# PKU-VCL-Geometry/GeoSplatting

Measured on AMD Instinct MI355X. Metric: fwd+bwd views/sec at 2M Gaussians, 800x800, higher is better.
Workload: dtype f32

## Files before the change

geosplatting_amd/_lib.py:

```python
from __future__ import annotations

import ctypes as C
import os
from typing import Optional

import torch

_HERE = os.path.dirname(os.path.abspath(__file__))
LIB_PATH = os.path.join(_HERE, "libgeosplat_hip.so")

GS_MAX_LEVELS = 16


class GsEnv(C.Structure):
    _fields_ = [("lut", C.c_void_p), ("lut_res", C.c_int), ("base", C.c_void_p), ("base_res", C.c_int),
                ("num_levels", C.c_int), ("levels", C.c_void_p * GS_MAX_LEVELS), ("res", C.c_int * GS_MAX_LEVELS),
                ("min_roughness", C.c_float), ("max_roughness", C.c_float)]


class GsTailView(C.Structure):
    _fields_ = [("viewmat", C.c_void_p), ("K", C.c_void_p), ("cam_pos", C.c_void_p), ("vis_records", C.c_void_p), ("v_packed", C.c_void_p),
                ("packed_index", C.c_void_p), ("W", C.c_int), ("H", C.c_int)]


class GsTileLevel(C.Structure):
    _fields_ = [("R", C.c_int), ("n_mirrors", C.c_int), ("margin", C.c_int), ("bw", C.c_int), ("nb", C.c_int), ("tile_begin", C.c_int),
                ("tile_end", C.c_int), ("reserved", C.c_int), ("src", C.c_void_p), ("scale", C.c_void_p), ("out_scale", C.c_void_p),
                ("bounds", C.c_void_p), ("tiles", C.c_void_p), ("segments", C.c_void_p), ("row_begin", C.c_void_p), ("row_counts", C.c_void_p),
                ("desc", C.c_void_p), ("weights", C.c_void_p), ("dst", C.c_void_p), ("lds_bytes", C.c_size_t)]


class GsEnvGrad(C.Structure):
    _fields_ = [("base", C.c_void_p), ("levels", C.c_void_p * GS_MAX_LEVELS)]


SYMBOLS = [
    "gs_last_error", "gs_version", "gs_project_ws_bytes", "gs_project_fwd", "gs_project_fwd_vis", "gs_project_fwd_vis_ex", "gs_isect_emit", "gs_sort_ws_bytes",
    "gs_isect_sort", "gs_isect_bin_ws_bytes", "gs_isect_bin", "gs_isect_offsets", "gs_raster_ws_bytes", "gs_raster_fwd", "gs_raster_prepare", "gs_raster_prepare_vis", "gs_raster_composite", "gs_raster_grad_stride", "gs_raster_bwd", "gs_raster_bwd_acc", "gs_selftest_rcp", "gs_selftest_exp", "gs_selftest_cube_edges", "gs_isect_bin_cap", "gs_isect_offsets_cap", "gs_isect_bin_tiles_cap", "gs_isect_offsets_tiles_cap", "gs_raster_prepare_vis_cap", "gs_raster_composite_cap", "gs_raster_bwd_cap", "gs_raster_bwd_acc_cap", "gs_raster_composite_tone", "gs_raster_bwd_tone_acc", "gs_raster_log_ws_bytes", "gs_raster_composite_tone_log", "gs_raster_bwd_tone_log_acc", "gs_project_bwd_cap", "gs_project_bwd", "gs_project_bwd_ex", "gs_shade_fwd",
    "gs_shade_bwd_ws_bytes", "gs_shade_bwd", "gs_tonemap_fwd", "gs_tonemap_bwd", "gs_tonemap_fwd3", "gs_tonemap_bwd3", "gs_cubemap_mip_fwd", "gs_cubemap_mip_chain_fwd", "gs_cube_sample_linear",
    "gs_cubemap_mip_bwd", "gs_diffuse_cubemap_fwd", "gs_diffuse_cubemap_bwd", "gs_specular_bounds", "gs_specular_bounds_ws_bytes", "gs_specular_bounds_fast", "gs_cube_dir_table",
    "gs_specular_cubemap_fwd", "gs_specular_cubemap_bwd", "gs_specular_tiles_count", "gs_specular_tiles_fill",
    "gs_specular_tiles_check", "gs_specular_tiles_apply", "gs_specular_tiles_apply_multi", "gs_mgadapter_fwd", "gs_mgadapter_bwd", "gs_vertex_normals_fwd",
    "gs_vertex_normals_bwd", "gs_photo_loss_ws_bytes", "gs_photo_loss", "gs_hashgrid_fwd", "gs_hashgrid_bwd_ws_bytes", "gs_hashgrid_bwd", "gs_hashgrid_bwd_fixed_ws_bytes", "gs_hashgrid_bwd_fixed", "gs_mlp_wgrad_ws_bytes", "gs_mlp_wgrad",
    "gs_flexicubes_ws_bytes", "gs_flexicubes_count", "gs_flexicubes_fwd", "gs_flexicubes_bwd", "gs_flexicubes_entropy_fwd",
    "gs_flexicubes_entropy_bwd", "gs_front_ws_bytes", "gs_front_fwd", "gs_isect_bin_front_ws_bytes", "gs_isect_bin_front", "gs_tail_bwd", "gs_tail_bwd_multi", "gs_tail_bwd_multi_parts", "gs_tail_priv_ws_bytes", "gs_tail_priv_reduce", "gs_activation_chain",
]

_lib: Optional[C.CDLL] = None


class GeoSplatHipError(RuntimeError):
    pass


def lib() -> C.CDLL:
    global _lib
    if _lib is None:
        if not os.path.exists(LIB_PATH):
            raise GeoSplatHipError(
                f"{LIB_PATH} not found: build it with `python -m geosplatting_amd.build` "
                "(hipcc --offload-arch=gfx950).  geosplatting_amd has no CPU / PyTorch fallback.")
        l = C.CDLL(LIB_PATH)
        l.gs_last_error.restype = C.c_char_p
        l.gs_project_ws_bytes.restype = C.c_size_t
        l.gs_project_ws_bytes.argtypes = [C.c_int]
        l.gs_sort_ws_bytes.restype = C.c_size_t
        l.gs_sort_ws_bytes.argtypes = [C.c_int64, C.c_int, C.c_int]
        l.gs_isect_bin_ws_bytes.restype = C.c_size_t
        l.gs_isect_bin_ws_bytes.argtypes = [C.c_int, C.c_int64, C.c_int, C.c_int]
        l.gs_shade_bwd_ws_bytes.restype = C.c_size_t
        l.gs_shade_bwd_ws_bytes.argtypes = [C.c_void_p, C.c_int]
        l.gs_hashgrid_bwd_ws_bytes.restype = C.c_size_t
        l.gs_hashgrid_bwd_ws_bytes.argtypes = [C.c_int, C.c_int, C.c_int]
        l.gs_hashgrid_bwd_fixed_ws_bytes.restype = C.c_size_t
        l.gs_hashgrid_bwd_fixed_ws_bytes.argtypes = [C.c_int, C.c_int, C.c_int, C.c_int]
        l.gs_mlp_wgrad_ws_bytes.restype = C.c_size_t
        l.gs_mlp_wgrad_ws_bytes.argtypes = [C.c_int64]
        l.gs_flexicubes_ws_bytes.restype = C.c_size_t
        l.gs_flexicubes_ws_bytes.argtypes = [C.c_int, C.c_int, C.c_int]
        l.gs_photo_loss_ws_bytes.restype = C.c_size_t
        l.gs_photo_loss_ws_bytes.argtypes = [C.c_int, C.c_int]
        l.gs_specular_bounds_ws_bytes.restype = C.c_size_t
        l.gs_specular_bounds_ws_bytes.argtypes = [C.c_int]
        l.gs_front_ws_bytes.restype = C.c_size_t
        l.gs_front_ws_bytes.argtypes = [C.c_int]
        l.gs_isect_bin_front_ws_bytes.restype = C.c_size_t
        l.gs_isect_bin_front_ws_bytes.argtypes = [C.c_int, C.c_int64, C.c_int, C.c_int]
        l.gs_tail_priv_ws_bytes.restype = C.c_size_t
        l.gs_tail_priv_ws_bytes.argtypes = [C.c_void_p, C.c_int]
        l.gs_raster_log_ws_bytes.restype = C.c_size_t
        l.gs_raster_log_ws_bytes.argtypes = [C.c_int64, C.c_int, C.c_int, C.c_int]
        l.gs_raster_ws_bytes.restype = C.c_size_t
        l.gs_raster_ws_bytes.argtypes = [C.c_int64, C.c_int, C.c_int, C.c_int, C.c_int]
        _lib = l
    return _lib


def check(rc: int, what: str) -> None:
    if rc != 0:
        raise GeoSplatHipError(f"{what} failed ({rc}): {lib().gs_last_error().decode()}")


def ptr(t: Optional[torch.Tensor]) -> Optional[C.c_void_p]:
    if t is None:
        return None
    assert t.is_cuda and t.is_contiguous(), "device-resident contiguous tensors only"
    return C.c_void_p(t.data_ptr())


def stream() -> C.c_void_p:
    return C.c_void_p(torch.cuda.current_stream().cuda_stream)


def f32(x: float) -> C.c_float:
    return C.c_float(float(x))


def i64(x: int) -> C.c_int64:
    return C.c_int64(int(x))


def require_cuda(*tensors: torch.Tensor) -> None:
    for t in tensors:
        if t is not None and not t.is_cuda:
            raise GeoSplatHipError("geosplatting_amd ops run on the GPU only (tensor on %s); there is no CPU path" % t.device)


_shared_streams = {}


def shared_stream(device: torch.device, role: str) -> "torch.cuda.Stream":
    key = (device.index if device.index is not None else torch.cuda.current_device(), role)
    st = _shared_streams.get(key)
    if st is None:
        st = _shared_streams[key] = torch.cuda.Stream(device=device)
    return st
```

geosplatting_amd/csrc/gs_common.h:

```cpp
#pragma once
#include <hip/hip_runtime.h>
#include <stdint.h>
#include <stdio.h>

#include "../../include/geosplat_hip.h"

#define GS_WAVE 64

void gs_set_error(const char* fmt, ...);

#define GS_CHECK_ARG(cond, msg)                                  \
    do {                                                         \
        if (!(cond)) { gs_set_error("%s: %s", __func__, msg); return GS_EINVAL; } \
    } while (0)

#define GS_CHECK_HIP(expr)                                                              \
    do {                                                                                \
        hipError_t _e = (expr);                                                         \
        if (_e != hipSuccess) {                                                         \
            gs_set_error("%s: %s failed: %s", __func__, #expr, hipGetErrorString(_e));  \
            return GS_ELAUNCH;                                                          \
        }                                                                               \
    } while (0)

#define GS_CHECK_LAUNCH()  GS_CHECK_HIP(hipGetLastError())

static inline int gs_cdiv(int64_t a, int64_t b) { return (int)((a + b - 1) / b); }

struct GsCount {
    long long n;
    const long long* dev;
};
__device__ __forceinline__ long long gs_count(const GsCount& c)
{
    if (c.dev == nullptr) return c.n;
    const long long v = *c.dev;
    return v < 0 ? 0 : (v < c.n ? v : c.n);
}

static __global__ void __launch_bounds__(256) gs_zero_kernel(uint32_t* __restrict__ p, size_t n_words)
{
    for (size_t i = (size_t)blockIdx.x * blockDim.x + threadIdx.x; i < n_words; i += (size_t)gridDim.x * blockDim.x) p[i] = 0u;
}
static __global__ void __launch_bounds__(256) gs_zero16_kernel(uint4* __restrict__ p, size_t n_quads)
{
    for (size_t i = (size_t)blockIdx.x * blockDim.x + threadIdx.x; i < n_quads; i += (size_t)gridDim.x * blockDim.x) p[i] = make_uint4(0u, 0u, 0u, 0u);
}
static inline hipError_t gs_zero_async(void* p, size_t bytes, hipStream_t s)
{
    if (bytes == 0) return hipSuccess;
    if ((bytes & 3) != 0 || (((uintptr_t)p) & 3) != 0) return hipMemsetAsync(p, 0, bytes, s);
    const bool wide = (bytes & 15) == 0 && (((uintptr_t)p) & 15) == 0;
    const size_t n = wide ? bytes / 16 : bytes / 4;
    const size_t want = (n + 255) / 256;
    const int blocks = (int)(want < 4096 ? want : 4096);
    if (wide) hipLaunchKernelGGL(gs_zero16_kernel, dim3(blocks), dim3(256), 0, s, (uint4*)p, n);
    else hipLaunchKernelGGL(gs_zero_kernel, dim3(blocks), dim3(256), 0, s, (uint32_t*)p, n);
    return hipGetLastError();
}

__device__ __forceinline__ float gs_readlane(float v, int lane)
{
    return __builtin_bit_cast(float, __builtin_amdgcn_readlane(__builtin_bit_cast(int, v), lane));
}
__device__ __forceinline__ int gs_readlane(int v, int lane) { return __builtin_amdgcn_readlane(v, lane); }

template <int CTRL, int ROW_MASK, int BANK_MASK>
__device__ __forceinline__ float gs_dpp_add(float v)
{
    int o = __builtin_amdgcn_update_dpp(0, __builtin_bit_cast(int, v), CTRL, ROW_MASK, BANK_MASK, false);
    return v + __builtin_bit_cast(float, o);
}

__device__ __forceinline__ float gs_wave_sum(float v)
{
    v = gs_dpp_add<0xB1, 0xf, 0xf>(v);
    v = gs_dpp_add<0x4E, 0xf, 0xf>(v);
    v = gs_dpp_add<0x141, 0xf, 0xf>(v);
    v = gs_dpp_add<0x140, 0xf, 0xf>(v);
    v = gs_dpp_add<0x142, 0xa, 0xf>(v);
    v = gs_dpp_add<0x143, 0xc, 0xf>(v);
    return gs_readlane(v, 63);
}

template <int CTRL, int ROW_MASK>
__device__ __forceinline__ unsigned gs_dpp_add_u32(unsigned v)
{
    return v + (unsigned)__builtin_amdgcn_update_dpp(0, (int)v, CTRL, ROW_MASK, 0xf, false);
}
__device__ __forceinline__ unsigned gs_wave_incl_scan(unsigned v)
{
    v = gs_dpp_add_u32<0x111, 0xf>(v);
    v = gs_dpp_add_u32<0x112, 0xf>(v);
    v = gs_dpp_add_u32<0x114, 0xf>(v);
    v = gs_dpp_add_u32<0x118, 0xf>(v);
    v = gs_dpp_add_u32<0x142, 0xa>(v);
    v = gs_dpp_add_u32<0x143, 0xc>(v);
    return v;
}
__device__ __forceinline__ int gs_wave_incl_scan(int v) { return (int)gs_wave_incl_scan((unsigned)v); }
__device__ __forceinline__ unsigned gs_wave_sum_u32(unsigned v)
{
    v = gs_dpp_add_u32<0xB1, 0xf>(v);
    v = gs_dpp_add_u32<0x4E, 0xf>(v);
    v = gs_dpp_add_u32<0x141, 0xf>(v);
    v = gs_dpp_add_u32<0x140, 0xf>(v);
    v = gs_dpp_add_u32<0x142, 0xa>(v);
    v = gs_dpp_add_u32<0x143, 0xc>(v);
    return (unsigned)__builtin_amdgcn_readlane((int)v, 63);
}
__device__ __forceinline__ unsigned long long gs_wave_sum_u64(unsigned long long v)
{
    const unsigned a = gs_wave_sum_u32((unsigned)(v & 0x1fffffull)), b = gs_wave_sum_u32((unsigned)((v >> 21) & 0x1fffffull)),
                   c = gs_wave_sum_u32((unsigned)(v >> 42));
    return (unsigned long long)a + ((unsigned long long)b << 21) + ((unsigned long long)c << 42);
}

template <int CTRL>
__device__ __forceinline__ float gs_dpp_take(float give)
{
    return __builtin_bit_cast(float, __builtin_amdgcn_update_dpp(0, __builtin_bit_cast(int, give), CTRL, 0xf, 0xf, true));
}

template <int N, int CTRL>
__device__ __forceinline__ void gs_bfly_stage(const float* in, float* out, bool own_hi)
{
#pragma unroll
    for (int z = 0; z < (N + 1) / 2; ++z) {
        const float lo = in[2 * z];
        const float hi = (2 * z + 1 < N) ? in[2 * z + 1] : 0.0f;
        const float keep = own_hi ? hi : lo;
        const float give = own_hi ? lo : hi;
        out[z] = keep + gs_dpp_take<CTRL>(give);
    }
}

template <int NV>
struct GsBfly {
    static constexpr int N1 = (NV + 1) / 2, N2 = (N1 + 1) / 2, N3 = (N2 + 1) / 2, N4 = (N3 + 1) / 2;
    __device__ static __forceinline__ int owned_index(int lane, int q)
    {
        return 16 * q + 8 * (lane & 1) + 4 * ((lane >> 1) & 1) + 2 * ((lane >> 2) & 1) + ((lane >> 3) & 1);
    }
    __device__ static __forceinline__ void reduce_rows(const float (&v)[NV], float (&out)[N4], int lane)
    {
        float a[N1], b[N2], c[N3];
        gs_bfly_stage<NV, 0x140>(v, a, (lane & 8) != 0);
        gs_bfly_stage<N1, 0x141>(a, b, (lane & 4) != 0);
        gs_bfly_stage<N2, 0x4E>(b, c, (lane & 2) != 0);
        gs_bfly_stage<N3, 0xB1>(c, out, (lane & 1) != 0);
    }
    __device__ static __forceinline__ void reduce(const float (&v)[NV], float (&out)[N4], int lane)
    {
        float a[N1], b[N2], c[N3];
        gs_bfly_stage<NV, 0x140>(v, a, (lane & 8) != 0);
        gs_bfly_stage<N1, 0x141>(a, b, (lane & 4) != 0);
        gs_bfly_stage<N2, 0x4E>(b, c, (lane & 2) != 0);
        gs_bfly_stage<N3, 0xB1>(c, out, (lane & 1) != 0);
#pragma unroll
        for (int q = 0; q < N4; ++q) {
            out[q] += __shfl_xor(out[q], 16, 64);
            out[q] += __shfl_xor(out[q], 32, 64);
        }
    }
};

__device__ __forceinline__ float gs_exp_neg(float sigma)
{
#pragma clang fp contract(off)
    const float y = sigma * -1.44269504f;
    const float yc = fminf(fmaxf(y, -126.0f), 126.0f);
    const float n = __builtin_rintf(yc);
    const float f = yc - n;
    float p = 0x1.41a6fep-13f;
    p = __builtin_fmaf(p, f, 0x1.5f44f0p-10f);
    p = __builtin_fmaf(p, f, 0x1.3b2dfep-7f);
    p = __builtin_fmaf(p, f, 0x1.c6aed6p-5f);
    p = __builtin_fmaf(p, f, 0x1.ebfbdap-3f);
    p = __builtin_fmaf(p, f, 0x1.62e430p-1f);
    p = __builtin_fmaf(p, f, 1.0f);
    const float r = __builtin_ldexpf(p, (int)n);
    return (y >= -125.0f) ? r : 0.0f;
}

__device__ __forceinline__ bool alpha_extent(float ca, float cb, float cc, float o, float& hx, float& hy)
{
    const float tau = __logf(255.0f * o);
    const float det = ca * cc - cb * cb;
    if (!(tau > -0.002f)) return false;
    if (!(det > 0.0f)) { hx = hy = 1e30f; return true; }
    const float k = 2.0f * (tau + 0.002f) / det;
    hx = sqrtf(k * cc) * 1.0005f + 0.02f;
    hy = sqrtf(k * ca) * 1.0005f + 0.02f;
    return true;
}

__device__ __forceinline__ void gs_write_vis_record(float4* __restrict__ rec, float mx, float my, float ca, float cb, float cc, float op,
                                                    float c0, float c1, float c2)
{
    float hx = -1.0f, hy = -1.0f;
    if (!alpha_extent(ca, cb, cc, op, hx, hy)) { hx = -1.0f; hy = -1.0f; }
    rec[0] = make_float4(mx, my, 0.5f * ca, cb);
    rec[1] = make_float4(0.5f * cc, op, hx, hy);
    rec[2] = make_float4(c0, c1, c2, 0.0f);
    rec[3] = make_float4(0.f, 0.f, 0.f, 0.f);
}

__device__ __forceinline__ int gs_lane_id() { return (int)(threadIdx.x & 63); }

__device__ __forceinline__ void gs_atomic_add(float* p, float v) { unsafeAtomicAdd(p, v); }

__device__ __forceinline__ void gs_atomic_add_xcd(float* p, float v)
{
    __hip_atomic_fetch_add(p, v, __ATOMIC_RELAXED, __HIP_MEMORY_SCOPE_WORKGROUP);
}

__device__ __forceinline__ int gs_xcc_id()
{
    return (int)(__builtin_amdgcn_s_getreg((3 << 11) | (0 << 6) | 20) & 0xf);
}
```

geosplatting_amd/csrc/gs_raster.hip:

```cpp
#include "gs_common.h"
#include "gs_tone.h"
#include <stdlib.h>

#pragma clang fp contract(off)

#define GS_TILE 16
#define GS_ALPHA_MIN (1.0f / 255.0f)

#ifdef GS_RASTER_STATS
__device__ unsigned long long g_raster_stats[8];
extern "C" int gs_raster_stats_read(unsigned long long* host8, int reset)
{
    if (hipMemcpyFromSymbol(host8, HIP_SYMBOL(g_raster_stats), sizeof(unsigned long long) * 8) != hipSuccess) return -1;
    if (reset) { unsigned long long z[8] = {0}; if (hipMemcpyToSymbol(HIP_SYMBOL(g_raster_stats), z, sizeof(z)) != hipSuccess) return -1; }
    return 0;
}
__device__ unsigned long long g_raster_stats2[8];
extern "C" int gs_raster_stats2_read(unsigned long long* host8, int reset)
{
    if (hipMemcpyFromSymbol(host8, HIP_SYMBOL(g_raster_stats2), sizeof(unsigned long long) * 8) != hipSuccess) return -1;
    if (reset) { unsigned long long z[8] = {0}; if (hipMemcpyToSymbol(HIP_SYMBOL(g_raster_stats2), z, sizeof(z)) != hipSuccess) return -1; }
    return 0;
}
__device__ unsigned long long g_raster_stats3[8];
// ... 1064 lines not shown
        GS_PHASE_BEGIN();
        lanes_lds_sync();
        qa[lane] = c0; qb[lane] = make_float2(c1.x, c1.y); qc[lane] = c2; qidx[lane] = c_idx;
        GS_STAT(5, nb);
        const int idx_low = __builtin_amdgcn_readlane(c_idx, nb - 1);
        const bool live = bin_final >= idx_low;
        const unsigned long long act = __ballot(live);
        const unsigned long long pm = lane < nb ? (c_msk & act) : 0ull;
        if (__ballot(pm != 0ull) == 0ull) { GS_PHASE_END(1); continue; }
        const float4 ra4 = c0;
        const float2 rb4 = make_float2(c1.x, c1.y);
        const int cnt = __popcll(pm);
        int cum = cnt;
        cum = gs_wave_incl_scan(cum);
        GS_PHASE_END(1);
        int r0 = 0, cumbase = 0;
        while (r0 < nb) {
            const int r1 = r0 + __popcll(__ballot(lane >= r0 && lane < nb && (cum - cumbase) <= GS_LOG_PAIR_CAP));
            const bool mine = lane >= r0 && lane < r1;
            const unsigned long long pms = mine ? pm : 0ull;
            lanes_lds_sync();
            msk[lane] = pms;
            pbase[lane] = cum - cnt - cumbase;
            unsigned long long list = gs_bit_transpose64(pms, lane);
#ifdef GS_RASTER_STATS
            GS_STAT2(1, 1);
            GS_STAT2_ALL(0, __popcll(list));
#endif
            lanes_lds_sync();
            long long _pw0 = 0;
#ifdef GS_RASTER_PHASES
            if (blockIdx.x == 0 && threadIdx.x == 0) { _pw0 = (long long)__builtin_readcyclecounter(); atomicAdd(&g_raster_stats[6], 1ull); }
#endif
            if (__ballot(list != 0ull) != 0ull) do {
                GS_STAT(6, 1);
#if defined(GS_RASTER_STATS) && !defined(GS_RASTER_PHASES)
                { const int na = __popcll(__ballot(list != 0ull));
#pragma unroll
                  for (int k = 0; k < 8; ++k) walk_hist[k] += (na > 8 * k && na <= 8 * k + 8) ? 1 : 0; }
#endif
#ifdef GS_RASTER_PHASES
                if (blockIdx.x == 0 && threadIdx.x == 0) atomicAdd(&g_raster_stats[5], 1ull);
#endif
#if GS_LOG_ASSIST_MAX > 0
                {
                    const unsigned long long am = __ballot(list != 0ull);
                    const int na = __popcll(am);
                    if (na <= GS_LOG_ASSIST_MAX && __ballot(__popcll(list) > 2) != 0ull) {
                        const int gs = na <= 8 ? 3 : 2, G = 1 << gs;
                        const int rank = __popcll(am & lane_lt);
                        lanes_lds_sync();
                        if (list != 0ull) apix[rank] = lane;
                        lanes_lds_sync();
                        const int g = lane >> gs, h = lane & (G - 1);
                        const bool grp = g < na;
                        const int p = grp ? apix[g] : 0;
                        const int pa = p << 2;
                        unsigned long long L = ((unsigned long long)(unsigned)__builtin_amdgcn_ds_bpermute(pa, (int)(unsigned)(list >> 32)) << 32) |
                                               (unsigned long long)(unsigned)__builtin_amdgcn_ds_bpermute(pa, (int)(unsigned)list);
                        const float T0 = __builtin_bit_cast(float, __builtin_amdgcn_ds_bpermute(pa, __builtin_bit_cast(int, T)));
                        const float Z0 = __builtin_bit_cast(float, __builtin_amdgcn_ds_bpermute(pa, __builtin_bit_cast(int, zacc)));
                        const int bf = __builtin_amdgcn_ds_bpermute(pa, bin_final);
                        float vr[CD];
#pragma unroll
                        for (int c = 0; c < CD; ++c) vr[c] = __builtin_bit_cast(float, __builtin_amdgcn_ds_bpermute(pa, __builtin_bit_cast(int, v_rc[c])));
                        if (!grp) L = 0ull;
                        for (int i = 0; i < G - 1; ++i) L = (i < h) ? (L & (L - 1ull)) : L;
                        const bool has = L != 0ull;
                        const int j = gs_pop_lowest(L);
                        const float4 a = qa[j]; const float2 b = qb[j]; const float4 cc = qc[j];
                        const int idx = qidx[j];
                        const unsigned long long below = (1ull << p) - 1ull;
                        const int e = pbase[j] + __popcll(msk[j] & below);
                        float sigma, ov, alpha, ra;
                        {
#pragma clang fp contract(off)
                            const v2f d = v2f{a.x, a.y} - v2f{(float)(qx0 + (p & 7)) + 0.5f, (float)(qy0 + (p >> 3)) + 0.5f};
                            const v2f pp = v2f{a.z, a.w} * v2f{d.x, d.x};
                            sigma = gs_sigma_xy(d, pp, b.x);
                            ov = b.y * __builtin_amdgcn_exp2f(sigma * -1.4426950408889634f);
                            alpha = fminf(ov, 0.999f);
                            const float x = 1.0f - alpha;
                            const float r0 = __builtin_amdgcn_rcpf(x);
                            ra = fmaf(r0, fmaf(-x, r0, 1.0f), r0);
                        }
                        const bool ok = has & (idx <= bf) & (sigma >= 0.0f) & (alpha >= GS_ALPHA_MIN);
                        float cv = cc.x * vr[0];
                        if (CD > 1) cv = fmaf(cc.y, vr[1], cv);
                        if (CD > 2) cv = fmaf(cc.z, vr[2], cv);
                        float pi = ok ? ra : 1.0f;
                        { const float t = gs_row_shr<0x111>(1.0f, pi); pi *= (h >= 1) ? t : 1.0f; }
                        { const float t = gs_row_shr<0x112>(1.0f, pi); pi *= (h >= 2) ? t : 1.0f; }
                        { const float t = gs_row_shr<0x114>(1.0f, pi); pi *= (h >= 4) ? t : 1.0f; }
                        float pe = gs_row_shr<0x111>(1.0f, pi); pe = (h >= 1) ? pe : 1.0f;
                        const float Tb = T0 * pe, Tn = Tb * ra;
                        const float fac = ok ? alpha * Tn : 0.0f;
                        float si = fac * cv;
                        { const float t = gs_row_shr<0x111>(0.0f, si); si += (h >= 1) ? t : 0.0f; }
                        { const float t = gs_row_shr<0x112>(0.0f, si); si += (h >= 2) ? t : 0.0f; }
                        { const float t = gs_row_shr<0x114>(0.0f, si); si += (h >= 4) ? t : 0.0f; }
                        float se = gs_row_shr<0x111>(0.0f, si); se = (h >= 1) ? se : 0.0f;
                        const float zb = Z0 - se;
                        const float v_alpha = fmaf(Tn, cv, ra * zb);
                        const float s_out = (ok && ov <= 0.999f) ? -ov * v_alpha : 0.0f;
#ifdef GS_RASTER_STATS
                        if (ok) GS_STAT_ALL(7, 1);
                        if (has && !ok) { if (idx > bf) GS_STAT2_ALL(2, 1); else GS_STAT2_ALL(3, 1); }
#endif
                        pairbuf[has ? e : GS_LOG_PAIR_CAP] = make_float2(s_out, fac);
                        const float T_end = T0 * pi, Z_end = Z0 - si;
                        const int src = (((rank << gs) + G - 1) & 63) << 2;
                        const float Tg = __builtin_bit_cast(float, __builtin_amdgcn_ds_bpermute(src, __builtin_bit_cast(int, T_end)));
                        const float Zg = __builtin_bit_cast(float, __builtin_amdgcn_ds_bpermute(src, __builtin_bit_cast(int, Z_end)));
                        const unsigned Llo = (unsigned)__builtin_amdgcn_ds_bpermute(src, (int)(unsigned)L);
                        const unsigned Lhi = (unsigned)__builtin_amdgcn_ds_bpermute(src, (int)(unsigned)(L >> 32));
                        if (list != 0ull) { T = Tg; zacc = Zg; list = ((unsigned long long)Lhi << 32) | Llo; }
                        continue;
                    }
                }
#endif
                const bool has0 = list != 0ull;
                const int j0 = gs_pop_lowest(list);
                const bool has1 = list != 0ull;
                const int j1 = gs_pop_lowest(list);
                const float4 a0 = qa[j0], a1 = qa[j1];
                const float2 b0 = qb[j0], b1 = qb[j1];
                const float4 cc0 = qc[j0], cc1 = qc[j1];
                const int idx0 = qidx[j0], idx1 = qidx[j1];
                const int e0 = pbase[j0] + __popcll(msk[j0] & lane_lt), e1 = pbase[j1] + __popcll(msk[j1] & lane_lt);
                v2f sigma, ov, alpha, ra;
                {
#pragma clang fp contract(off)
                    const v2f d0 = v2f{a0.x, a0.y} - pxy, d1 = v2f{a1.x, a1.y} - pxy;
                    const v2f p0 = v2f{a0.z, a0.w} * v2f{d0.x, d0.x}, p1 = v2f{a1.z, a1.w} * v2f{d1.x, d1.x};
                    sigma.x = gs_sigma_xy(d0, p0, b0.x);
                    sigma.y = gs_sigma_xy(d1, p1, b1.x);
#ifndef GS_BWD_LOG_EXACT_MATH
                    ov = v2f{b0.y, b1.y} * v2f{__builtin_amdgcn_exp2f(sigma.x * -1.4426950408889634f), __builtin_amdgcn_exp2f(sigma.y * -1.4426950408889634f)};
                    alpha = __builtin_elementwise_min(ov, (v2f)(0.999f));
                    {
                        const v2f x = (v2f)(1.0f) - alpha;
                        const v2f r0 = v2f{__builtin_amdgcn_rcpf(x.x), __builtin_amdgcn_rcpf(x.y)};
                        ra = __builtin_elementwise_fma(r0, __builtin_elementwise_fma(-x, r0, (v2f)(1.0f)), r0);
                    }
#else
                    ov = v2f{b0.y, b1.y} * gs_exp_neg_live2(sigma);
                    alpha = __builtin_elementwise_min(ov, (v2f)(0.999f));
                    ra = gs_rcp_exact2((v2f)(1.0f) - alpha);
#endif
                }
                const bool ok0 = has0 & (idx0 <= bin_final) & (sigma.x >= 0.0f) & (alpha.x >= GS_ALPHA_MIN);
                const bool ok1 = has1 & (idx1 <= bin_final) & (sigma.y >= 0.0f) & (alpha.y >= GS_ALPHA_MIN);
                {
                    const float Tn = T * ra.x;
                    const float fac = ok0 ? alpha.x * Tn : 0.0f;
                    float cv = cc0.x * v_rc[0];
                    if (CD > 1) cv = fmaf(cc0.y, v_rc[1], cv);
                    if (CD > 2) cv = fmaf(cc0.z, v_rc[2], cv);
                    const float v_alpha = fmaf(Tn, cv, ra.x * zacc);
                    const float s_out = (ok0 && ov.x <= 0.999f) ? -ov.x * v_alpha : 0.0f;
                    zacc = fmaf(-fac, cv, zacc);
                    T = ok0 ? Tn : T;
#ifdef GS_RASTER_STATS
                    if (ok0) GS_STAT_ALL(7, 1);
                    if (has0 && !ok0) { if (idx0 > bin_final) GS_STAT2_ALL(2, 1); else GS_STAT2_ALL(3, 1); }
#endif
                    pairbuf[has0 ? e0 : GS_LOG_PAIR_CAP] = make_float2(s_out, fac);
                }
                {
                    const float Tn = T * ra.y;
                    const float fac = ok1 ? alpha.y * Tn : 0.0f;
                    float cv = cc1.x * v_rc[0];
                    if (CD > 1) cv = fmaf(cc1.y, v_rc[1], cv);
                    if (CD > 2) cv = fmaf(cc1.z, v_rc[2], cv);
                    const float v_alpha = fmaf(Tn, cv, ra.y * zacc);
                    const float s_out = (ok1 && ov.y <= 0.999f) ? -ov.y * v_alpha : 0.0f;
                    zacc = fmaf(-fac, cv, zacc);
                    T = ok1 ? Tn : T;
#ifdef GS_RASTER_STATS
                    if (ok1) GS_STAT_ALL(7, 1);
                    if (has1 && !ok1) { if (idx1 > bin_final) GS_STAT2_ALL(2, 1); else GS_STAT2_ALL(3, 1); }
#endif
                    pairbuf[has1 ? e1 : GS_LOG_PAIR_CAP] = make_float2(s_out, fac);
                }
            } while (__ballot(list != 0ull) != 0ull);
            lanes_lds_sync();
#ifdef GS_RASTER_PHASES
            if (blockIdx.x == 0 && threadIdx.x == 0) { const long long _t = (long long)__builtin_readcyclecounter(); atomicAdd(&g_raster_stats[2], (unsigned long long)(_t - _pw0)); _pw0 = _t; }
#endif
            float sum[NV];
            {
                const float X = ra4.x - ((float)qx0 + 0.5f), Y = ra4.y - ((float)qy0 + 0.5f);
                unsigned long long m = pms;
                int e = cum - cnt - cumbase;
                float m0 = 0.0f, mxy = 0.0f, c2s = 0.0f;
                v2f m1 = (v2f)(0.0f), m2 = (v2f)(0.0f), c01 = (v2f)(0.0f);
                if (__ballot(m != 0ull) != 0ull) do {
                    GS_STAT2(7, 1);
#ifdef GS_RASTER_PHASES
                    if (blockIdx.x == 0 && threadIdx.x == 0) atomicAdd(&g_raster_stats[7], 1ull);
#endif
                    const bool has = m != 0ull;
                    const int p = gs_pop_lowest(m);
                    const float2 sfr = pairbuf[has ? e : 0];
                    float4 vr;
                    vr.x = __shfl(v_rc[0], p, 64); vr.y = CD > 1 ? __shfl(v_rc[1], p, 64) : 0.0f; vr.z = CD > 2 ? __shfl(v_rc[2], p, 64) : 0.0f; vr.w = 0.0f;
                    e += has ? 1 : 0;
                    const float s_w = has ? sfr.x : 0.0f, f_w = has ? sfr.y : 0.0f;
                    const v2f d = v2f{X, Y} - v2f{(float)(p & 7), (float)(p >> 3)};
                    const v2f sd = d * s_w;
                    m0 += s_w;
                    m1 += sd;
                    m2 = __builtin_elementwise_fma(sd, d, m2);
                    mxy = fmaf(sd.x, d.y, mxy);
                    c01 = __builtin_elementwise_fma((v2f)(f_w), v2f{vr.x, vr.y}, c01);
                    if (CD > 2) c2s = fmaf(f_w, vr.z, c2s);
                } while (__ballot(m != 0ull) != 0ull);
                sum[0] = m0; sum[1] = m1.x; sum[2] = m1.y; sum[3] = m2.x; sum[4] = mxy; sum[5] = m2.y;
                sum[6] = c01.x;
                if (CD > 1) sum[7] = c01.y;
                if (CD > 2) sum[8] = c2s;
            }
            lanes_lds_sync();
#ifdef GS_RASTER_PHASES
            if (blockIdx.x == 0 && threadIdx.x == 0) { const long long _t = (long long)__builtin_readcyclecounter(); atomicAdd(&g_raster_stats[3], (unsigned long long)(_t - _pw0)); _pw0 = _t; }
#endif
            {
                const float ga = ra4.z, gb = ra4.w, gc = rb4.x, go = rb4.y;
                const float M0 = sum[0], Mx = sum[1], My = sum[2];
                float out[NV];
                out[0] = (2.0f * ga) * Mx + gb * My;
                out[1] = gb * Mx + (2.0f * gc) * My;
                out[2] = 0.5f * sum[3]; out[3] = sum[4]; out[4] = 0.5f * sum[5];
                out[5] = (M0 != 0.0f) ? -M0 / go : 0.0f;
#pragma unroll
                for (int k = 0; k < CD; ++k) out[6 + k] = sum[6 + k];
                if (mine) {
#pragma unroll
                    for (int k = 0; k < NV; ++k) stage[lane * NV + k] = out[k];
                }
            }
            lanes_lds_sync();
            {
                const int r = lane / NV, k = lane - r * NV;
                for (int it = 0; r0 + it * RPI < r1; ++it) {
                    const int j = r0 + it * RPI + r;
                    if (r < RPI && j < r1 && k < 6 + D) {
                        const float v = stage[j * NV + k];
                        if (v != 0.0f) {
                            const int g = __float_as_int(qc[j].w);
                            gs_atomic_add(v_packed + (size_t)g * rec_stride + k, v);
                        }
                    }
                }
            }
#ifdef GS_RASTER_PHASES
            if (blockIdx.x == 0 && threadIdx.x == 0) atomicAdd(&g_raster_stats[4], (unsigned long long)((long long)__builtin_readcyclecounter() - _pw0));
#endif
            cumbase = __builtin_amdgcn_readlane(cum, r1 - 1);
            r0 = r1;
        }
    }
#if defined(GS_RASTER_STATS) && !defined(GS_RASTER_PHASES)
    if (lane == 0) {
#pragma unroll
        for (int k = 0; k < 8; ++k) if (walk_hist[k]) atomicAdd(&g_raster_stats3[k], (unsigned long long)walk_hist[k]);
    }
#endif
    GS_TL_END();
}

#define GS_RASTER_BLOCKS_PER_CU 4
static int gs_raster_blocks_per_cu() { return GS_RASTER_BLOCKS_PER_CU; }
static size_t gs_raster_lds_pad() { return (size_t)(160 * 1024 / gs_raster_blocks_per_cu()) - 1024; }
static size_t gs_raster_lds(size_t natural)
{
    const size_t pad = gs_raster_lds_pad();
    if (natural >= pad) return natural;
    if ((size_t)(gs_raster_blocks_per_cu() + 1) * (natural + 512) > (size_t)160 * 1024) return natural;
    return pad;
}
static size_t align256(size_t x) { return (x + 255) & ~(size_t)255; }

extern "C" size_t gs_raster_ws_bytes(int64_t n_isects, int V, int W, int H, int tile_size)
{
    if (tile_size <= 0) return 0;
    const size_t tiles = (size_t)((W + tile_size - 1) / tile_size) * (size_t)((H + tile_size - 1) / tile_size);
    const size_t n = n_isects > 0 ? (size_t)n_isects : 1;
    const size_t v = V > 0 ? (size_t)V : 1;
    return 3 * align256(n * sizeof(float4)) + align256(tiles * sizeof(int32_t)) + align256(64 * sizeof(int32_t)) +
           align256(64 * tiles * sizeof(int32_t)) + align256(4 * v * sizeof(float4));
}

struct RasterWs {
    float4 *rec0, *rec1, *rec2;
    int32_t* order;
    BwdOrder bo;
    float4* vis;
};
static RasterWs carve(void* ws, int64_t n_isects, int V, int tiles)
{
    const size_t n = n_isects > 0 ? (size_t)n_isects : 1;
    const size_t v = V > 0 ? (size_t)V : 1;
    char* p = (char*)ws;
    RasterWs r;
    r.rec0 = (float4*)p; p += align256(n * sizeof(float4));
    r.rec1 = (float4*)p; p += align256(n * sizeof(float4));
    r.rec2 = (float4*)p; p += align256(n * sizeof(float4));
    r.order = (int32_t*)p; p += align256((size_t)tiles * sizeof(int32_t));
    r.bo.bcount = (int32_t*)p; p += align256(64 * sizeof(int32_t));
    r.bo.blist = (int32_t*)p; p += align256(64 * (size_t)tiles * sizeof(int32_t));
    r.vis = (float4*)p;
    return r;
}

struct RasterOpts {
    const int64_t* counts = nullptr;
    ToneFwd tone_fwd = { 0, nullptr, nullptr };
    ToneBwd tone_bwd = { 0, nullptr, nullptr, nullptr, nullptr };
    CullLog log = { nullptr, nullptr, nullptr };
};
static GsCount isect_count(int64_t n, const RasterOpts& o)
{
    return GsCount{ (long long)n, o.counts ? (const long long*)o.counts + 1 : nullptr };
}

template <int CD>
static int launch_fwd(int W, int H, int D, const RasterWs& ws, const float* colors, const float* background,
                      int64_t n_isects, const int32_t* offsets, float* render, float* alphas, int32_t* last_ids,
                      hipStream_t s, const RasterOpts& o)
{
    const int tile_w = (W + GS_TILE - 1) / GS_TILE, tile_h = (H + GS_TILE - 1) / GS_TILE;
    if (o.tone_fwd.image && !(CD == 3 && D == 3 && background == nullptr)) {
        gs_set_error("gs_raster_composite_tone: needs D == 3 and no background");
        return GS_EINVAL;
    }
    {
        const size_t planes = CD > 3 ? 4 * (size_t)2 * (size_t)D * 64 * sizeof(float) : 0;
        const size_t lds = gs_raster_lds(4 * (size_t)GS_WIN_Q_BYTES + planes);
        if (lds > 64 * 1024)
            GS_CHECK_HIP(hipFuncSetAttribute((const void*)raster_fwd_window_kernel<CD>, hipFuncAttributeMaxDynamicSharedMemorySize, (int)lds));
        hipLaunchKernelGGL(raster_fwd_window_kernel<CD>, dim3(tile_w * tile_h), dim3(256), lds, s, W, H, tile_w, tile_w * tile_h, D,
                           ws.order, ws.rec0, ws.rec1, ws.rec2, colors, background, isect_count(n_isects, o), offsets, render, alphas,
                           last_ids, o.tone_fwd, o.log, o.log.count ? ws.bo : BwdOrder{ nullptr, nullptr });
        GS_CHECK_LAUNCH();
        return GS_OK;
    }
}

static int raster_check(const char* who, int W, int H, int tile_size, int D, int V, int64_t n_isects, const void* ws,
                        size_t ws_bytes)
{
    GS_CHECK_ARG(W > 0 && H > 0, "bad image size");
    GS_CHECK_ARG(tile_size == GS_TILE, "only tile_size=16 is built (rfstudio/model/gsplat.py:30)");
    GS_CHECK_ARG(D >= 1 && D <= GS_MAX_CHANNELS, "1 <= D <= 32");
    GS_CHECK_ARG(n_isects >= 0 && n_isects < (1ll << 31), "n_isects must fit int32");
    GS_CHECK_ARG(ws != nullptr, "workspace must not be NULL");
    GS_CHECK_ARG(V >= 0, "bad V");
    if (ws_bytes < gs_raster_ws_bytes(n_isects, V, W, H, tile_size)) { gs_set_error("%s: workspace too small", who); return GS_ENOSPC; }
    return GS_OK;
}

static int raster_prepare_impl(int W, int H, int tile_size, int D, int V, const float* means2d, const float* conics,
                               const float* opacities, const float* colors, const float* vis_records, int64_t n_isects,
                               const int32_t* offsets, const int32_t* flatten_ids, void* ws, size_t ws_bytes, void* stream,
                               const RasterOpts& o)
{
    const int rc = raster_check("gs_raster_prepare", W, H, tile_size, D, V, n_isects, ws, ws_bytes);
    if (rc != GS_OK) return rc;
    hipStream_t s = (hipStream_t)stream;
    const int tiles = ((W + GS_TILE - 1) / GS_TILE) * ((H + GS_TILE - 1) / GS_TILE);
    const RasterWs r = carve(ws, n_isects, V, tiles);
    if (n_isects > 0 && V > 0) {
        const float4* vis = (const float4*)vis_records;
        if (!vis) {
            hipLaunchKernelGGL(pack_visible_kernel, dim3(gs_cdiv(V, 256)), dim3(256), 0, s, V, D, means2d, conics, opacities, colors,
                               r.vis);
            GS_CHECK_LAUNCH();
            vis = r.vis;
        }
        hipLaunchKernelGGL(build_stream_packed_kernel, dim3(gs_cdiv(n_isects, 256)), dim3(256), 0, s, isect_count(n_isects, o), flatten_ids,
                           vis, r.rec0, r.rec1, r.rec2);
        GS_CHECK_LAUNCH();
    }
    hipLaunchKernelGGL(tile_order_kernel, dim3(1), dim3(1024), 0, s, tiles, isect_count(n_isects, o), offsets, r.order, r.bo);
    GS_CHECK_LAUNCH();
    return GS_OK;
}

static int raster_composite_impl(int W, int H, int tile_size, int D, int V, const float* colors, const float* background,
                                 int64_t n_isects, const int32_t* offsets, float* render, float* alphas, int32_t* last_ids,
                                 const void* ws, size_t ws_bytes, void* stream, const RasterOpts& o)
{
    const int rc = raster_check("gs_raster_composite", W, H, tile_size, D, V, n_isects, ws, ws_bytes);
    if (rc != GS_OK) return rc;
    hipStream_t s = (hipStream_t)stream;
    const int tiles = ((W + GS_TILE - 1) / GS_TILE) * ((H + GS_TILE - 1) / GS_TILE);
    const RasterWs r = carve((void*)ws, n_isects, V, tiles);
#define GS_FWD(CD) return launch_fwd<CD>(W, H, D, r, colors, background, n_isects, offsets, render, alphas, last_ids, s, o)
    if (D <= 3) GS_FWD(3);
    if (D <= 4) GS_FWD(4);
    if (D <= 8) GS_FWD(8);
    if (D <= 16) GS_FWD(16);
    GS_FWD(32);
#undef GS_FWD
}

template <int CD>
static int launch_bwd(int W, int H, int D, const RasterWs& ws, const float* colors, const float* background,
                      int64_t n_isects, const int32_t* offsets, const float* alphas, const int32_t* last_ids,
                      const float* v_render, const float* v_alphas, float* v_packed, int rec_stride, hipStream_t s,
                      const RasterOpts& o)
{
    const int tile_w = (W + GS_TILE - 1) / GS_TILE, tile_h = (H + GS_TILE - 1) / GS_TILE;
    if (o.tone_bwd.v_image && !(CD == 3 && D == 3 && background == nullptr)) {
        gs_set_error("gs_raster_bwd_tone: needs D == 3 and no background");
        return GS_EINVAL;
    }
    if constexpr (CD <= 3) {
        if (o.log.idx) {
            const size_t lds = gs_raster_lds(4 * (size_t)LogLds::WAVE_BYTES);
            hipLaunchKernelGGL(raster_bwd_log_kernel<CD>, dim3(tile_w * tile_h), dim3(256), lds, s, W, H, tile_w, tile_w * tile_h, D,
                               ws.order, ws.rec0, ws.rec1, ws.rec2, background, isect_count(n_isects, o), offsets, alphas, last_ids,
                               v_render, v_alphas, v_packed, rec_stride, o.tone_bwd, o.log, ws.bo);
            GS_CHECK_LAUNCH();
            return GS_OK;
        }
    }
    {
        size_t lds = 4 * ((size_t)Lanes2Lds<CD>::WAVE_BYTES + (CD > 3 ? 2 * (size_t)D * 64 * 4 : 0));
        if (lds < gs_raster_lds_pad()) lds = gs_raster_lds_pad();
        if (lds > 64 * 1024)
            GS_CHECK_HIP(hipFuncSetAttribute((const void*)raster_bwd_lanes2_kernel<CD>, hipFuncAttributeMaxDynamicSharedMemorySize, (int)lds));
        hipLaunchKernelGGL(raster_bwd_lanes2_kernel<CD>, dim3(tile_w * tile_h), dim3(256), lds, s, W, H, tile_w, tile_w * tile_h, D,
                           ws.order, ws.rec0, ws.rec1, ws.rec2, colors, background, isect_count(n_isects, o), offsets, alphas, last_ids,
                           v_render, v_alphas, v_packed, rec_stride, o.tone_bwd);
        GS_CHECK_LAUNCH();
        return GS_OK;
    }
}

extern "C" int gs_raster_grad_stride(int D) { return ((6 + D) + 15) / 16 * 16; }

static int raster_bwd_impl(int W, int H, int tile_size, int D, int V, const float* colors, const float* background,
                           int64_t n_isects, const int32_t* offsets, const float* alphas, const int32_t* last_ids,
                           const float* v_render, const float* v_alphas, float* v_packed, const void* ws,
                           size_t ws_bytes, void* stream, bool zero, const RasterOpts& o)
{
    const int rc = raster_check("gs_raster_bwd", W, H, tile_size, D, V, n_isects, ws, ws_bytes);
    if (rc != GS_OK) return rc;
    hipStream_t s = (hipStream_t)stream;
    const int rec_stride = gs_raster_grad_stride(D);
    if (V > 0 && zero) GS_CHECK_HIP(gs_zero_async(v_packed, sizeof(float) * (size_t)rec_stride * (size_t)V, s));
    if (n_isects == 0 || V == 0) return GS_OK;
    const int tiles = ((W + GS_TILE - 1) / GS_TILE) * ((H + GS_TILE - 1) / GS_TILE);
    const RasterWs r = carve((void*)ws, n_isects, V, tiles);
#define GS_BWD(CD) return launch_bwd<CD>(W, H, D, r, colors, background, n_isects, offsets, alphas, last_ids, v_render, v_alphas, v_packed, rec_stride, s, o)
    if (D <= 3) GS_BWD(3);
    if (D <= 4) GS_BWD(4);
    if (D <= 8) GS_BWD(8);
    if (D <= 16) GS_BWD(16);
    GS_BWD(32);
#undef GS_BWD
}

static CullLog carve_log(const void* log_ws, int64_t n_isects)
{
    const size_t n = n_isects > 0 ? (size_t)n_isects : 1;
    char* p = (char*)log_ws;
    CullLog l;
    l.mask = (unsigned long long*)p; p += align256(4 * n * sizeof(unsigned long long));
    l.idx = (int32_t*)p; p += align256(4 * n * sizeof(int32_t));
    l.count = (int32_t*)p;
    return l;
}
extern "C" size_t gs_raster_log_ws_bytes(int64_t n_isects, int W, int H, int tile_size)
{
    if (tile_size <= 0) return 0;
    const size_t n = n_isects > 0 ? (size_t)n_isects : 1;
    const size_t tiles = (size_t)((W + tile_size - 1) / tile_size) * (size_t)((H + tile_size - 1) / tile_size);
    return align256(4 * n * sizeof(unsigned long long)) + align256(4 * n * sizeof(int32_t)) + align256(4 * tiles * sizeof(int32_t));
}

extern "C" int gs_raster_prepare(int W, int H, int tile_size, int D, int V, const float* means2d, const float* conics,
                                 const float* opacities, const float* colors, int64_t n_isects, const int32_t* offsets,
                                 const int32_t* flatten_ids, void* ws, size_t ws_bytes, void* stream)
{
    return raster_prepare_impl(W, H, tile_size, D, V, means2d, conics, opacities, colors, nullptr, n_isects, offsets, flatten_ids,
                               ws, ws_bytes, stream, RasterOpts{});
}

extern "C" int gs_raster_prepare_vis(int W, int H, int tile_size, int D, int V, const float* vis_records, int64_t n_isects,
                                     const int32_t* offsets, const int32_t* flatten_ids, void* ws, size_t ws_bytes, void* stream)
{
    GS_CHECK_ARG(vis_records != nullptr || V == 0, "vis_records (written by gs_project_fwd_vis) must not be NULL");
    return raster_prepare_impl(W, H, tile_size, D, V, nullptr, nullptr, nullptr, nullptr, vis_records, n_isects, offsets,
                               flatten_ids, ws, ws_bytes, stream, RasterOpts{});
}

extern "C" int gs_raster_composite(int W, int H, int tile_size, int D, int V, const float* colors, const float* background,
                                   int64_t n_isects, const int32_t* offsets, float* render, float* alphas,
                                   int32_t* last_ids, const void* ws, size_t ws_bytes, void* stream)
{
    return raster_composite_impl(W, H, tile_size, D, V, colors, background, n_isects, offsets, render, alphas, last_ids, ws,
                                 ws_bytes, stream, RasterOpts{});
}

extern "C" int gs_raster_fwd(int W, int H, int tile_size, int D, int V, const float* means2d, const float* conics,
                             const float* opacities, const float* colors, const float* background,
                             int64_t n_isects, const int32_t* offsets, const int32_t* flatten_ids,
                             float* render, float* alphas, int32_t* last_ids, void* ws, size_t ws_bytes, void* stream)
{
    const int rc = raster_prepare_impl(W, H, tile_size, D, V, means2d, conics, opacities, colors, nullptr, n_isects, offsets,
                                       flatten_ids, ws, ws_bytes, stream, RasterOpts{});
    if (rc != GS_OK) return rc;
    return raster_composite_impl(W, H, tile_size, D, V, colors, background, n_isects, offsets, render, alphas, last_ids, ws,
                                 ws_bytes, stream, RasterOpts{});
}

extern "C" int gs_raster_bwd(int W, int H, int tile_size, int D, int V, const float* colors, const float* background,
                             int64_t n_isects, const int32_t* offsets, const float* alphas, const int32_t* last_ids,
                             const float* v_render, const float* v_alphas, float* v_packed, const void* ws,
                             size_t ws_bytes, void* stream)
{
    return raster_bwd_impl(W, H, tile_size, D, V, colors, background, n_isects, offsets, alphas, last_ids, v_render, v_alphas,
                           v_packed, ws, ws_bytes, stream, true, RasterOpts{});
}

extern "C" int gs_raster_bwd_acc(int W, int H, int tile_size, int D, int V, const float* colors, const float* background,
                                 int64_t n_isects, const int32_t* offsets, const float* alphas, const int32_t* last_ids,
                                 const float* v_render, const float* v_alphas, float* v_packed, const void* ws,
                                 size_t ws_bytes, void* stream)
{
    return raster_bwd_impl(W, H, tile_size, D, V, colors, background, n_isects, offsets, alphas, last_ids, v_render, v_alphas,
                           v_packed, ws, ws_bytes, stream, false, RasterOpts{});
}

extern "C" int gs_raster_prepare_vis_cap(int W, int H, int tile_size, int D, int V_cap, const float* vis_records, int64_t n_isects_cap,
                                         const int64_t* counts_dev, const int32_t* offsets, const int32_t* flatten_ids, void* ws,
                                         size_t ws_bytes, void* stream)
{
    GS_CHECK_ARG(counts_dev != nullptr, "counts_dev must not be NULL");
    GS_CHECK_ARG(vis_records != nullptr || V_cap == 0, "vis_records (written by gs_project_fwd_vis) must not be NULL");
    RasterOpts o;
    o.counts = counts_dev;
    return raster_prepare_impl(W, H, tile_size, D, V_cap, nullptr, nullptr, nullptr, nullptr, vis_records, n_isects_cap, offsets,
                               flatten_ids, ws, ws_bytes, stream, o);
}

extern "C" int gs_raster_composite_cap(int W, int H, int tile_size, int D, int V_cap, const float* colors, const float* background,
                                       int64_t n_isects_cap, const int64_t* counts_dev, const int32_t* offsets, float* render,
                                       float* alphas, int32_t* last_ids, const void* ws, size_t ws_bytes, void* stream)
{
    GS_CHECK_ARG(counts_dev != nullptr, "counts_dev must not be NULL");
    RasterOpts o;
    o.counts = counts_dev;
    return raster_composite_impl(W, H, tile_size, D, V_cap, colors, background, n_isects_cap, offsets, render, alphas, last_ids, ws,
                                 ws_bytes, stream, o);
}

extern "C" int gs_raster_bwd_cap(int W, int H, int tile_size, int D, int V_cap, const float* colors, const float* background,
                                 int64_t n_isects_cap, const int64_t* counts_dev, const int32_t* offsets, const float* alphas,
                                 const int32_t* last_ids, const float* v_render, const float* v_alphas, float* v_packed, const void* ws,
                                 size_t ws_bytes, void* stream)
{
    GS_CHECK_ARG(counts_dev != nullptr, "counts_dev must not be NULL");
    RasterOpts o;
    o.counts = counts_dev;
    return raster_bwd_impl(W, H, tile_size, D, V_cap, colors, background, n_isects_cap, offsets, alphas, last_ids, v_render, v_alphas,
                           v_packed, ws, ws_bytes, stream, true, o);
}

extern "C" int gs_raster_bwd_acc_cap(int W, int H, int tile_size, int D, int V_cap, const float* colors, const float* background,
                                     int64_t n_isects_cap, const int64_t* counts_dev, const int32_t* offsets, const float* alphas,
                                     const int32_t* last_ids, const float* v_render, const float* v_alphas, float* v_packed,
                                     const void* ws, size_t ws_bytes, void* stream)
{
    GS_CHECK_ARG(counts_dev != nullptr, "counts_dev must not be NULL");
    RasterOpts o;
    o.counts = counts_dev;
    return raster_bwd_impl(W, H, tile_size, D, V_cap, colors, background, n_isects_cap, offsets, alphas, last_ids, v_render, v_alphas,
                           v_packed, ws, ws_bytes, stream, false, o);
}

extern "C" int gs_raster_composite_tone(int W, int H, int tile_size, int V, const float* colors, int64_t n_isects,
                                        const int64_t* counts_dev, const int32_t* offsets, float* render, float* alphas,
                                        int32_t* last_ids, int tone_mode, const float* exposure, float* image, const void* ws,
                                        size_t ws_bytes, void* stream)
{
    GS_CHECK_ARG(tone_mode >= 0 && tone_mode <= 2 && exposure != nullptr && image != nullptr, "bad tone mode / exposure / image");
    RasterOpts o;
    o.counts = counts_dev;
    o.tone_fwd = ToneFwd{ tone_mode, exposure, (float4*)image };
    return raster_composite_impl(W, H, tile_size, 3, V, colors, nullptr, n_isects, offsets, render, alphas, last_ids, ws, ws_bytes,
                                 stream, o);
}

extern "C" int gs_raster_bwd_tone_acc(int W, int H, int tile_size, int V, const float* colors, int64_t n_isects,
                                      const int64_t* counts_dev, const int32_t* offsets, const float* render, const float* alphas,
                                      const int32_t* last_ids, int tone_mode, const float* exposure, const float* v_image,
                                      float* v_packed, float* v_exposure, const void* ws, size_t ws_bytes, void* stream)
{
    GS_CHECK_ARG(tone_mode >= 0 && tone_mode <= 2 && exposure != nullptr && v_image != nullptr && render != nullptr && v_exposure != nullptr,
                 "bad tone mode / exposure / v_image / render / v_exposure");
    RasterOpts o;
    o.counts = counts_dev;
    o.tone_bwd = ToneBwd{ tone_mode, exposure, render, (const float4*)v_image, v_exposure };
    return raster_bwd_impl(W, H, tile_size, 3, V, colors, nullptr, n_isects, offsets, alphas, last_ids, nullptr, nullptr, v_packed, ws,
                           ws_bytes, stream, false, o);
}

extern "C" int gs_raster_composite_tone_log(int W, int H, int tile_size, int V, const float* colors, int64_t n_isects,
                                            const int64_t* counts_dev, const int32_t* offsets, float* render, float* alphas,
                                            int32_t* last_ids, int tone_mode, const float* exposure, float* image, const void* ws,
                                            size_t ws_bytes, void* log_ws, size_t log_bytes, void* stream)
{
    GS_CHECK_ARG(log_ws != nullptr && tile_size == GS_TILE, "log_ws must not be NULL");
    if (log_bytes < gs_raster_log_ws_bytes(n_isects, W, H, tile_size)) { gs_set_error("gs_raster_composite_tone_log: log workspace too small"); return GS_ENOSPC; }
    GS_CHECK_ARG(tone_mode >= 0 && tone_mode <= 2 && exposure != nullptr && image != nullptr, "bad tone mode / exposure / image");
    RasterOpts o;
    o.counts = counts_dev;
    o.tone_fwd = ToneFwd{ tone_mode, exposure, (float4*)image };
    o.log = carve_log(log_ws, n_isects);
    return raster_composite_impl(W, H, tile_size, 3, V, colors, nullptr, n_isects, offsets, render, alphas, last_ids, ws, ws_bytes,
                                 stream, o);
}

extern "C" int gs_raster_bwd_tone_log_acc(int W, int H, int tile_size, int V, const float* colors, int64_t n_isects,
                                          const int64_t* counts_dev, const int32_t* offsets, const float* render, const float* alphas,
                                          const int32_t* last_ids, int tone_mode, const float* exposure, const float* v_image,
                                          float* v_packed, float* v_exposure, const void* ws, size_t ws_bytes, const void* log_ws,
                                          size_t log_bytes, void* stream)
{
    GS_CHECK_ARG(log_ws != nullptr && tile_size == GS_TILE, "log_ws must not be NULL");
    if (log_bytes < gs_raster_log_ws_bytes(n_isects, W, H, tile_size)) { gs_set_error("gs_raster_bwd_tone_log_acc: log workspace too small"); return GS_ENOSPC; }
    GS_CHECK_ARG(tone_mode >= 0 && tone_mode <= 2 && exposure != nullptr && v_image != nullptr && render != nullptr && v_exposure != nullptr,
                 "bad tone mode / exposure / v_image / render / v_exposure");
    RasterOpts o;
    o.counts = counts_dev;
    o.tone_bwd = ToneBwd{ tone_mode, exposure, render, (const float4*)v_image, v_exposure };
    o.log = carve_log(log_ws, n_isects);
    return raster_bwd_impl(W, H, tile_size, 3, V, colors, nullptr, n_isects, offsets, alphas, last_ids, nullptr, nullptr, v_packed, ws,
                           ws_bytes, stream, false, o);
}


__global__ void __launch_bounds__(256) selftest_rcp_kernel(uint32_t lo_bits, uint32_t hi_bits, unsigned long long* mismatches)
{
    const uint64_t n = (uint64_t)hi_bits - lo_bits + 1;
    unsigned long long bad = 0;
    for (uint64_t i = (uint64_t)blockIdx.x * blockDim.x + threadIdx.x; i < n; i += (uint64_t)gridDim.x * blockDim.x) {
        const float x = __uint_as_float(lo_bits + (uint32_t)i);
        const v2f r = gs_rcp_exact2(v2f{x, x});
        const float d = __fdiv_rn(1.0f, x);
        bad += (__float_as_uint(r.x) != __float_as_uint(d)) + (__float_as_uint(r.y) != __float_as_uint(d));
    }
    if (bad) atomicAdd(mismatches, bad);
}

extern "C" int gs_selftest_rcp(uint32_t lo_bits, uint32_t hi_bits, uint64_t* mismatches_dev, void* stream)
{
    GS_CHECK_ARG(mismatches_dev != nullptr && hi_bits >= lo_bits, "bad range");
    hipStream_t s = (hipStream_t)stream;
    GS_CHECK_HIP(gs_zero_async(mismatches_dev, sizeof(uint64_t), s));
    hipLaunchKernelGGL(selftest_rcp_kernel, dim3(4096), dim3(256), 0, s, lo_bits, hi_bits, (unsigned long long*)mismatches_dev);
    GS_CHECK_LAUNCH();
    return GS_OK;
}

__global__ void __launch_bounds__(256) selftest_exp_kernel(uint32_t lo_bits, uint32_t hi_bits, unsigned long long* out)
{
    const uint64_t n = (uint64_t)hi_bits - lo_bits + 1;
    unsigned long long sum = 0;
    double worst = 0.0;
    for (uint64_t i = (uint64_t)blockIdx.x * blockDim.x + threadIdx.x; i < n; i += (uint64_t)gridDim.x * blockDim.x) {
        const float x = __uint_as_float(lo_bits + (uint32_t)i);
        const float r = gs_exp_neg(x);
        sum += (unsigned long long)__float_as_uint(r) * (2ull * i + 1ull);
        const double ref = exp(-(double)x);
        const double e = fabs((double)r - ref) / ref;
        worst = e > worst ? e : worst;
    }
    atomicAdd(out, sum);
    atomicMax(out + 1, (unsigned long long)__double_as_longlong(worst));
}

extern "C" int gs_selftest_exp(uint32_t lo_bits, uint32_t hi_bits, uint64_t* out_dev, void* stream)
{
    GS_CHECK_ARG(out_dev != nullptr && hi_bits >= lo_bits, "bad range");
    hipStream_t s = (hipStream_t)stream;
    GS_CHECK_HIP(gs_zero_async(out_dev, 2 * sizeof(uint64_t), s));
    hipLaunchKernelGGL(selftest_exp_kernel, dim3(4096), dim3(256), 0, s, lo_bits, hi_bits, (unsigned long long*)out_dev);
    GS_CHECK_LAUNCH();
    return GS_OK;
}
```

geosplatting_amd/csrc/gs_sort.hip:

```cpp
#include "gs_common.h"

#include <cstdlib>
#include <cstring>

#define RS_THREADS 256
#define RS_WAVES 4
#define RS_ITEMS 8
#define RS_TILE (RS_THREADS * RS_ITEMS)
#define RS_WCHUNK (64 * RS_ITEMS)

typedef unsigned long long u64;

static int tile_bits(int tile_w, int tile_h)
{
    unsigned n = (unsigned)(tile_w * tile_h);
    int b = 0;
    while (n > 1) { n >>= 1; ++b; }
    return b + 1;
}

struct PairItem { u64 key; int32_t val; };
struct PairIn {
    const u64* keys; const int32_t* vals;
    __device__ __forceinline__ PairItem load(int64_t i) const { return PairItem{ keys[i], vals[i] }; }
};
struct PairOut {
    u64* keys; int32_t* vals;
    __device__ __forceinline__ void store(int64_t i, const PairItem& it) const { keys[i] = it.key; vals[i] = it.val; }
};
struct PairDigit {
    int shift; unsigned mask;
    __device__ __forceinline__ unsigned operator()(const PairItem& it) const { return (unsigned)(it.key >> shift) & mask; }
};

struct U2In {
    const uint2* p;
    __device__ __forceinline__ uint2 load(int64_t i) const { return p[i]; }
};
struct U2Out {
    uint2* p;
    __device__ __forceinline__ void store(int64_t i, const uint2& it) const { p[i] = it; }
};
struct DepthIn {
    const float* depths;
    __device__ __forceinline__ uint2 load(int64_t i) const { return make_uint2(__float_as_uint(depths[i]), (unsigned)i); }
};
struct XDigit {
    int shift; unsigned mask;
    __device__ __forceinline__ unsigned operator()(const uint2& it) const { return (it.x >> shift) & mask; }
};
struct FinalTiles {
    int32_t* tile_ids; int32_t* flatten_ids;
    __device__ __forceinline__ void store(int64_t i, const uint2& it) const
    {
        flatten_ids[i] = (int32_t)it.y;
        tile_ids[i] = (int32_t)it.x;
    }
};
struct FinalOut {
    u64* isect_ids; int32_t* flatten_ids; const float* depths;
    __device__ __forceinline__ void store(int64_t i, const uint2& it) const
    {
        flatten_ids[i] = (int32_t)it.y;
        isect_ids[i] = ((u64)it.x << 32) | (u64)__float_as_uint(depths[it.y]);
    }
};

template <typename Item, typename In, typename Digit>
__global__ void __launch_bounds__(RS_THREADS)
radix_hist_kernel(GsCount nc, In in, Digit digit, int nbins, int nblocks, unsigned* __restrict__ table)
{
    const int64_t n = gs_count(nc);
    __shared__ unsigned hist[256];
    hist[threadIdx.x] = 0u;
    __syncthreads();
    const int64_t base = (int64_t)blockIdx.x * RS_TILE;
#pragma unroll 4
    for (int k = 0; k < RS_ITEMS; ++k) {
        const int64_t i = base + (int64_t)k * RS_THREADS + threadIdx.x;
        if (i < n) atomicAdd(&hist[digit(in.load(i))], 1u);
    }
    __syncthreads();
    if ((int)threadIdx.x < nbins) table[(size_t)threadIdx.x * nblocks + blockIdx.x] = hist[threadIdx.x];
}

__global__ void __launch_bounds__(256)
radix_rowscan_kernel(int nblocks, unsigned* __restrict__ table, unsigned* __restrict__ row_total)
{
    __shared__ unsigned wsum[4];
    unsigned* row = table + (size_t)blockIdx.x * nblocks;
    const int lane = threadIdx.x & 63, wave = threadIdx.x >> 6;
    unsigned carry = 0u;
    for (int i0 = 0; i0 < nblocks; i0 += 256) {
        const int i = i0 + threadIdx.x;
        const unsigned v = i < nblocks ? row[i] : 0u;
        unsigned incl = v;
        incl = gs_wave_incl_scan(incl);
        if (lane == 63) wsum[wave] = incl;
        __syncthreads();
        unsigned before = 0u, all = 0u;
        for (int w = 0; w < 4; ++w) { if (w < wave) before += wsum[w]; all += wsum[w]; }
        if (i < nblocks) row[i] = carry + before + incl - v;
        carry += all;
        __syncthreads();
    }
    if (threadIdx.x == 0) row_total[blockIdx.x] = carry;
}

template <typename Item, typename In, typename Digit, typename Out, int NBITS>
__global__ void __launch_bounds__(RS_THREADS)
radix_scatter_kernel(GsCount nc, In in, Digit digit, int nblocks, const unsigned* __restrict__ table,
                     const unsigned* __restrict__ row_total, Out out)
{
    const int64_t n = gs_count(nc);
    constexpr int NB = 1 << NBITS;
    __shared__ unsigned cnt[RS_WAVES][NB];
    __shared__ unsigned dstart[NB];
    __shared__ unsigned gbase[NB];
    __shared__ Item stage[RS_TILE];
    const int lane = threadIdx.x & 63, wave = threadIdx.x >> 6;
    for (int i = threadIdx.x; i < RS_WAVES * NB; i += RS_THREADS) (&cnt[0][0])[i] = 0u;
    __syncthreads();
    const int64_t bbase = (int64_t)blockIdx.x * RS_TILE;
    const int64_t wbase = bbase + (int64_t)wave * RS_WCHUNK;
    const int n_here = (n - bbase) < RS_TILE ? (int)((n - bbase) > 0 ? (n - bbase) : 0) : RS_TILE;
    const u64 lane_lt = (1ull << lane) - 1ull;
    Item item[RS_ITEMS];
    unsigned dig[RS_ITEMS];
    unsigned rank[RS_ITEMS];
#pragma unroll
    for (int k = 0; k < RS_ITEMS; ++k) {
        const int64_t i = wbase + (int64_t)k * 64 + lane;
        const bool valid = i < n;
        if (valid) item[k] = in.load(i);
        const unsigned d = valid ? digit(item[k]) : 0u;
        u64 m = __ballot(valid);
#pragma unroll
        for (int b = 0; b < NBITS; ++b) {
            const bool bit = (d >> b) & 1u;
            const u64 bal = __ballot(bit);
            m &= bit ? bal : ~bal;
        }
        const unsigned old = cnt[wave][d];
        __builtin_amdgcn_wave_barrier();
        const unsigned r = __popcll(m & lane_lt);
        if (valid && r == 0u) cnt[wave][d] = old + (unsigned)__popcll(m);
        __builtin_amdgcn_fence(__ATOMIC_RELEASE, "wavefront");
        __builtin_amdgcn_wave_barrier();
        __builtin_amdgcn_fence(__ATOMIC_ACQUIRE, "wavefront");
        dig[k] = d;
        rank[k] = old + r;
    }
    __syncthreads();
    {
        const int d = threadIdx.x;
        unsigned tot = 0u;
        if (d < NB) for (int w = 0; w < RS_WAVES; ++w) tot += cnt[w][d];
        unsigned incl = tot;
        incl = gs_wave_incl_scan(incl);
        __shared__ unsigned wtot[RS_WAVES];
        if (lane == 63) wtot[wave] = incl;
        __syncthreads();
        unsigned before = 0u;
        for (int w = 0; w < wave; ++w) before += wtot[w];
        if (d < NB) dstart[d] = before + incl - tot;
        __syncthreads();
        const unsigned rt = d < NB ? row_total[d] : 0u;
        unsigned rincl = rt;
        rincl = gs_wave_incl_scan(rincl);
        if (lane == 63) wtot[wave] = rincl;
        __syncthreads();
        unsigned rbefore = 0u;
        for (int w = 0; w < wave; ++w) rbefore += wtot[w];
        if (d < NB) gbase[d] = rbefore + rincl - rt + table[(size_t)d * nblocks + blockIdx.x];
    }
    __syncthreads();
#pragma unroll
    for (int k = 0; k < RS_ITEMS; ++k) {
        const int64_t i = wbase + (int64_t)k * 64 + lane;
        if (i < n) {
            const unsigned d = dig[k];
            unsigned off = dstart[d] + rank[k];
            for (int w = 0; w < wave; ++w) off += cnt[w][d];
            stage[off] = item[k];
        }
    }
    __syncthreads();
#pragma unroll 4
    for (int k = 0; k < RS_ITEMS; ++k) {
        const int p = k * RS_THREADS + (int)threadIdx.x;
        if (p < n_here) {
            const Item it = stage[p];
            const unsigned d = digit(it);
            out.store((int64_t)gbase[d] + (int64_t)(p - (int)dstart[d]), it);
        }
    }
}

template <typename Item, typename In, typename Digit, typename Out>
static int radix_pass(GsCount nc, In in, Digit digit, Out out, int nbits, unsigned* table, hipStream_t s)
{
    const int64_t n = nc.n;
    const int nblocks = (int)((n + RS_TILE - 1) / RS_TILE);
    const int nbins = 1 << nbits;
    unsigned* row_total = table + (size_t)256 * nblocks;
    hipLaunchKernelGGL((radix_hist_kernel<Item, In, Digit>), dim3(nblocks), dim3(RS_THREADS), 0, s, nc, in, digit, nbins, nblocks, table);
    GS_CHECK_LAUNCH();
    hipLaunchKernelGGL(radix_rowscan_kernel, dim3(nbins), dim3(256), 0, s, nblocks, table, row_total);
    GS_CHECK_LAUNCH();
    switch (nbits) {
#define RS_CASE(B) case B: hipLaunchKernelGGL((radix_scatter_kernel<Item, In, Digit, Out, B>), dim3(nblocks), dim3(RS_THREADS), 0, s, nc, in, digit, nblocks, table, row_total, out); break;
        RS_CASE(1) RS_CASE(2) RS_CASE(3) RS_CASE(4) RS_CASE(5) RS_CASE(6) RS_CASE(7) RS_CASE(8)
#undef RS_CASE
        default: gs_set_error("radix_pass: bad digit width %d", nbits); return GS_EINVAL;
    }
    GS_CHECK_LAUNCH();
    return GS_OK;
}

static size_t align256(size_t x) { return (x + 255) & ~(size_t)255; }
static size_t table_bytes(int64_t n) { return align256(((size_t)256 * (size_t)((n + RS_TILE - 1) / RS_TILE + 1) + 512) * sizeof(unsigned)); }

extern "C" size_t gs_sort_ws_bytes(int64_t n_isects, int tile_w, int tile_h)
{
    if (n_isects <= 0) return 0;
    (void)tile_w; (void)tile_h;
    return table_bytes(n_isects) + align256((size_t)n_isects * 8) + align256((size_t)n_isects * 4) + 256;
}

extern "C" int gs_isect_sort(int64_t n_isects, const int64_t* isect_ids, const int32_t* flatten_ids,
                             int64_t* isect_ids_sorted, int32_t* flatten_ids_sorted, int tile_w, int tile_h,
                             void* ws, size_t ws_bytes, void* stream)
{
    GS_CHECK_ARG(n_isects >= 0 && tile_w > 0 && tile_h > 0, "bad sizes");
    if (n_isects == 0) return GS_OK;
    GS_CHECK_ARG(ws != nullptr, "workspace must not be NULL");
    if (ws_bytes < gs_sort_ws_bytes(n_isects, tile_w, tile_h)) { gs_set_error("gs_isect_sort: workspace too small"); return GS_ENOSPC; }
    hipStream_t s = (hipStream_t)stream;
    char* p = (char*)ws;
    unsigned* table = (unsigned*)p; p += table_bytes(n_isects);
    u64* tk = (u64*)p; p += align256((size_t)n_isects * 8);
    int32_t* tv = (int32_t*)p;
    const int end_bit = 32 + tile_bits(tile_w, tile_h);
    const int npass = (end_bit + 7) / 8;
    const u64* src_k = (const u64*)isect_ids; const int32_t* src_v = flatten_ids;
    for (int pass = 0; pass < npass; ++pass) {
        const int shift = pass * 8;
        const int nbits = (end_bit - shift) < 8 ? (end_bit - shift) : 8;
        const bool to_out = ((npass - 1 - pass) % 2) == 0;
        u64* dk = to_out ? (u64*)isect_ids_sorted : tk;
        int32_t* dv = to_out ? flatten_ids_sorted : tv;
        const int rc = radix_pass<PairItem>(GsCount{ n_isects, nullptr }, PairIn{ src_k, src_v }, PairDigit{ shift, (1u << nbits) - 1u }, PairOut{ dk, dv }, nbits, table, s);
        if (rc != GS_OK) return rc;
        src_k = dk; src_v = dv;
    }
    return GS_OK;
}

__device__ __forceinline__ void tile_range_sorted(float mx, float my, int radius, int tile_size, int tw, int th,
                                                  int& x0, int& y0, int& x1, int& y1)
{
#pragma clang fp contract(off)
    const float ts = (float)tile_size;
    const float tr = (float)radius / ts;
    const float tx = mx / ts, ty = my / ts;
    const float fx0 = floorf(tx - tr), fy0 = floorf(ty - tr);
    const float fx1 = ceilf(tx + tr), fy1 = ceilf(ty + tr);
    x0 = fx0 < 0.0f ? 0 : (fx0 > (float)tw ? tw : (int)fx0);
    y0 = fy0 < 0.0f ? 0 : (fy0 > (float)th ? th : (int)fy0);
    x1 = fx1 < 0.0f ? 0 : (fx1 > (float)tw ? tw : (int)fx1);
    y1 = fy1 < 0.0f ? 0 : (fy1 > (float)th ? th : (int)fy1);
}

#define EM_THREADS 256
#define EM_PER 4
#define EM_LOOK 4
#define EM_TILE (EM_THREADS * EM_PER)

__global__ void __launch_bounds__(256)
tile_rect_kernel(GsCount vc, const float* __restrict__ means2d, const int32_t* __restrict__ radii, int tile_size, int tile_w, int tile_h,
                 uint2* __restrict__ rect)
{
    const int V = (int)gs_count(vc);
    const int v = blockIdx.x * blockDim.x + threadIdx.x;
    if (v >= V) return;
    const float2 m = *reinterpret_cast<const float2*>(means2d + 2 * (size_t)v);
    int x0 = 0, y0 = 0, x1 = 0, y1 = 0;
    const int r = radii[v];
    if (r > 0) tile_range_sorted(m.x, m.y, r, tile_size, tile_w, tile_h, x0, y0, x1, y1);
    rect[v] = make_uint2((unsigned)x0 | ((unsigned)y0 << 16), (unsigned)x1 | ((unsigned)y1 << 16));
}
__device__ __forceinline__ unsigned rect_count(uint2 q)
{
    const int w = (int)(q.y & 0xffffu) - (int)(q.x & 0xffffu), h = (int)(q.y >> 16) - (int)(q.x >> 16);
    return (w > 0 && h > 0) ? (unsigned)(w * h) : 0u;
}

static size_t bf_state_bytes(int V) { return align256(16 + 2 * (size_t)((V + EM_TILE - 1) / EM_TILE + 1) * sizeof(u64)); }

extern "C" size_t gs_isect_bin_ws_bytes(int V, int64_t n_isects, int tile_w, int tile_h)
{
    (void)tile_w; (void)tile_h;
    const size_t v = V > 0 ? (size_t)V : 1, n = n_isects > 0 ? (size_t)n_isects : 1;
    const size_t tb = table_bytes((int64_t)(v > n ? v : n));
    return tb + 3 * align256(v * 8) + bf_state_bytes((int)v) + 2 * align256(n * 8) + 256;
}

__global__ void capacity_check_kernel(const long long* __restrict__ counts, long long v_cap, long long i_cap, long long* __restrict__ status)
{
    if (threadIdx.x != 0 || blockIdx.x != 0) return;
    const long long V = counts[0], I = counts[1];
    if (V > v_cap || I > i_cap) {
        status[0] = GS_ENOSPC;
        if (I > status[1]) status[1] = I;
        if (V > status[2]) status[2] = V;
    }
}

static int isect_bin_impl(int V, const float* means2d, const int32_t* radii, const float* depths, int64_t n_isects,
                          const long long* counts_dev, int tile_size, int tile_w, int tile_h, int64_t* isect_ids_sorted,
                          int32_t* flatten_ids_sorted, void* ws, size_t ws_bytes, void* stream, int32_t* tile_ids_sorted);

extern "C" int gs_isect_bin(int V, const float* means2d, const int32_t* radii, const float* depths,
                            const int32_t* tiles_per_gauss, int64_t n_isects, int tile_size, int tile_w, int tile_h,
                            int64_t* isect_ids_sorted, int32_t* flatten_ids_sorted, void* ws, size_t ws_bytes, void* stream)
{
    (void)tiles_per_gauss;
    return isect_bin_impl(V, means2d, radii, depths, n_isects, nullptr, tile_size, tile_w, tile_h, isect_ids_sorted, flatten_ids_sorted,
                          ws, ws_bytes, stream, nullptr);
}

extern "C" int gs_isect_bin_cap(int V_cap, const float* means2d, const int32_t* radii, const float* depths, const int64_t* counts_dev,
                                int64_t n_isects_cap, int tile_size, int tile_w, int tile_h, int64_t* isect_ids_sorted,
                                int32_t* flatten_ids_sorted, void* ws, size_t ws_bytes, int64_t* status_dev, void* stream)
{
    GS_CHECK_ARG(counts_dev != nullptr && status_dev != nullptr, "counts_dev / status_dev must not be NULL");
    hipLaunchKernelGGL(capacity_check_kernel, dim3(1), dim3(64), 0, (hipStream_t)stream, (const long long*)counts_dev, (long long)V_cap,
                       (long long)n_isects_cap, (long long*)status_dev);
    GS_CHECK_LAUNCH();
    return isect_bin_impl(V_cap, means2d, radii, depths, n_isects_cap, (const long long*)counts_dev, tile_size, tile_w, tile_h,
                          isect_ids_sorted, flatten_ids_sorted, ws, ws_bytes, stream, nullptr);
}

extern "C" int gs_isect_bin_tiles_cap(int V_cap, const float* means2d, const int32_t* radii, const float* depths, const int64_t* counts_dev,
                                      int64_t n_isects_cap, int tile_size, int tile_w, int tile_h, int32_t* tile_ids_sorted,
                                      int32_t* flatten_ids_sorted, void* ws, size_t ws_bytes, int64_t* status_dev, void* stream)
{
    GS_CHECK_ARG(counts_dev != nullptr && status_dev != nullptr && tile_ids_sorted != nullptr, "counts_dev / status_dev / tile_ids_sorted must not be NULL");
    hipLaunchKernelGGL(capacity_check_kernel, dim3(1), dim3(64), 0, (hipStream_t)stream, (const long long*)counts_dev, (long long)V_cap,
                       (long long)n_isects_cap, (long long*)status_dev);
    GS_CHECK_LAUNCH();
    return isect_bin_impl(V_cap, means2d, radii, depths, n_isects_cap, (const long long*)counts_dev, tile_size, tile_w, tile_h,
                          nullptr, flatten_ids_sorted, ws, ws_bytes, stream, tile_ids_sorted);
}

struct KeyIn {
    const unsigned* keys;
    __device__ __forceinline__ uint2 load(int64_t i) const { return make_uint2(keys[i], (unsigned)i); }
};
struct FinalFlat {
    int32_t* flatten_ids;
    __device__ __forceinline__ void store(int64_t i, const uint2& it) const { flatten_ids[i] = (int32_t)it.y; }
};

#define BF_HIST_MAX 8192

__global__ void __launch_bounds__(256)
bin_setup_kernel(unsigned* __restrict__ state, int n_state_words,
                 const long long* __restrict__ counts, long long v_cap, long long i_cap, long long* __restrict__ status)
{
    const int i = blockIdx.x * blockDim.x + threadIdx.x, stride = gridDim.x * blockDim.x;
    for (int k = i; k < n_state_words; k += stride) state[k] = 0u;
    if (i == 0 && counts != nullptr && status != nullptr) {
        const long long V = counts[0], I = counts[1];
        if (V > v_cap || I > i_cap) {
            status[0] = GS_ENOSPC;
            if (I > status[1]) status[1] = I;
            if (V > status[2]) status[2] = V;
        }
    }
}

#define BF_VALID (1ull << 63)
#define BF_SPIN_LIMIT (1 << 22)

__global__ void __launch_bounds__(EM_THREADS)
emit_chained_kernel(GsCount vc, const uint2* __restrict__ order, const uint2* __restrict__ rect, unsigned* __restrict__ ctrl,
                    u64* __restrict__ desc, int n_blocks, int tile_w, uint2* __restrict__ items, unsigned item_cap,
                    long long* __restrict__ status )
{
    const int V = (int)gs_count(vc);
    __shared__ unsigned ws[EM_THREADS / 64];
    __shared__ unsigned s_block;
    __shared__ unsigned long long s_base;
    const int lane = threadIdx.x & 63, wave = threadIdx.x >> 6;
    if (threadIdx.x == 0) s_block = atomicAdd(ctrl, 1u);
    __syncthreads();
    const int block = (int)s_block;
    u64* agg = desc; u64* pre = desc + n_blocks;
    const int r0 = block * EM_TILE + (int)threadIdx.x * EM_PER;
    int v[EM_PER]; unsigned c[EM_PER]; uint2 q[EM_PER];
    unsigned mine = 0u;
#pragma unroll
    for (int k = 0; k < EM_PER; ++k) {
        const int r = r0 + k;
        v[k] = r < V ? (int)order[r].y : -1;
        q[k] = v[k] >= 0 ? rect[v[k]] : make_uint2(0u, 0u);
        c[k] = rect_count(q[k]);
        mine += c[k];
    }
    unsigned incl = mine;
    incl = gs_wave_incl_scan(incl);
    if (lane == 63) ws[wave] = incl;
    __syncthreads();
    unsigned before = 0u, total = 0u;
    for (int w = 0; w < EM_THREADS / 64; ++w) { if (w < wave) before += ws[w]; total += ws[w]; }
    if (wave == 0) {
        unsigned long long acc = 0ull;
        if (block > 0) {
            if (lane == 0) __hip_atomic_store(&agg[block], (u64)total | BF_VALID, __ATOMIC_RELAXED, __HIP_MEMORY_SCOPE_AGENT);
            int pos = block - 1;
            bool done = false;
            while (!done) {
                u64 pv[EM_LOOK], av[EM_LOOK];
#pragma unroll
                for (int j = 0; j < EM_LOOK; ++j) {
                    const int idx = pos - 64 * j - lane;
                    pv[j] = av[j] = 0ull;
                    if (idx >= 0) {
                        pv[j] = __hip_atomic_load(&pre[idx], __ATOMIC_RELAXED, __HIP_MEMORY_SCOPE_AGENT);
                        av[j] = __hip_atomic_load(&agg[idx], __ATOMIC_RELAXED, __HIP_MEMORY_SCOPE_AGENT);
                    }
                }
#pragma unroll
                for (int j = 0; j < EM_LOOK; ++j) {
                    if (done) break;
                    const int idx = pos - 64 * j - lane;
                    bool isP = idx < 0;
                    u64 val = 0ull;
                    if (idx >= 0) {
                        int spins = 0;
                        for (;;) {
                            if (pv[j] & BF_VALID) { isP = true; val = pv[j]; break; }
                            if (av[j] & BF_VALID) { val = av[j]; break; }
                            if (++spins > BF_SPIN_LIMIT) { atomicExch(ctrl + 1, 1u); if (status) status[0] = GS_ENOSPC; break; }
                            __builtin_amdgcn_s_sleep(2);
                            pv[j] = __hip_atomic_load(&pre[idx], __ATOMIC_RELAXED, __HIP_MEMORY_SCOPE_AGENT);
                            av[j] = __hip_atomic_load(&agg[idx], __ATOMIC_RELAXED, __HIP_MEMORY_SCOPE_AGENT);
                        }
                    }
                    const u64 pmask = __ballot(isP);
                    const int first = pmask ? __builtin_ctzll(pmask) : 64;
                    if (lane <= first) acc += val & ~BF_VALID;
                    if (pmask) done = true;
                }
                pos -= 64 * EM_LOOK;
            }
        }
        const unsigned long long base = gs_wave_sum_u64(acc);
        if (lane == 0) {
            __hip_atomic_store(&pre[block], (u64)(base + total) | BF_VALID, __ATOMIC_RELAXED, __HIP_MEMORY_SCOPE_AGENT);
            s_base = base;
        }
    }
    __syncthreads();
    unsigned long long cur = s_base + before + incl - mine;
#pragma unroll
    for (int k = 0; k < EM_PER; ++k) {
        if (v[k] < 0 || c[k] == 0u) continue;
        const int x0 = (int)(q[k].x & 0xffffu), y0 = (int)(q[k].x >> 16), x1 = (int)(q[k].y & 0xffffu), y1 = (int)(q[k].y >> 16);
        for (int i = y0; i < y1; ++i)
            for (int j = x0; j < x1; ++j) {
                const unsigned t = (unsigned)(i * tile_w + j);
                if (cur < (unsigned long long)item_cap) items[cur] = make_uint2(t, (unsigned)v[k]);
                ++cur;
            }
    }
}

__global__ void __launch_bounds__(1024)
tile_offsets_scan_kernel(int n_tiles, const unsigned* __restrict__ tile_counts, GsCount nc, int32_t* __restrict__ offsets)
{
    __shared__ unsigned wsum[16];
    const unsigned n = (unsigned)gs_count(nc);
    const int lane = threadIdx.x & 63, wave = threadIdx.x >> 6;
    unsigned carry = 0u;
    for (int i0 = 0; i0 < n_tiles; i0 += 1024) {
        const int i = i0 + threadIdx.x;
        const unsigned v = i < n_tiles ? tile_counts[i] : 0u;
        unsigned incl = v;
        incl = gs_wave_incl_scan(incl);
        if (lane == 63) wsum[wave] = incl;
        __syncthreads();
        unsigned before = 0u, all = 0u;
        for (int w = 0; w < 16; ++w) { if (w < wave) before += wsum[w]; all += wsum[w]; }
        if (i < n_tiles) { const unsigned o = carry + before + incl - v; offsets[i] = (int32_t)(o < n ? o : n); }
        carry += all;
        __syncthreads();
    }
}

__global__ void __launch_bounds__(256)
bin_offsets_tiles_kernel(GsCount nc, const int32_t* __restrict__ tiles, int n_tiles, int32_t* __restrict__ offsets)
{
    const int64_t n = gs_count(nc);
    const int64_t i = (int64_t)blockIdx.x * blockDim.x + threadIdx.x;
    if (n == 0 && i == 0)
        for (int t = 0; t < n_tiles; ++t) offsets[t] = 0;
    if (i >= n) return;
    const int cur = tiles[i];
    if (i == 0) {
        for (int t = 0; t <= cur && t < n_tiles; ++t) offsets[t] = 0;
    } else {
        const int prev = tiles[i - 1];
        for (int t = prev + 1; t <= cur && t < n_tiles; ++t) offsets[t] = (int32_t)i;
    }
    if (i == n - 1)
        for (int t = cur + 1; t < n_tiles; ++t) offsets[t] = (int32_t)n;
}


extern "C" size_t gs_isect_bin_front_ws_bytes(int V, int64_t n_isects, int tile_w, int tile_h)
{
    const size_t v = V > 0 ? (size_t)V : 1, n = n_isects > 0 ? (size_t)n_isects : 1;
    const size_t tb = table_bytes((int64_t)(v > n ? v : n));
    return tb + 2 * align256(v * 8) + 2 * align256(n * 8) + bf_state_bytes((int)v) + align256(n * 4) + 256;
}

extern "C" int gs_isect_bin_front(int V_cap, const uint32_t* depth_keys, const uint32_t* tile_rects, const uint32_t* tile_counts,
                                  const int64_t* counts_dev, int64_t n_isects_cap, int key_bits, int tile_w, int tile_h, int32_t* flatten_ids_sorted,
                                  int32_t* isect_offsets, void* ws, size_t ws_bytes, int64_t* status_dev, void* stream)
{
    const int V = V_cap;
    const int64_t n_isects = n_isects_cap;
    GS_CHECK_ARG(V >= 0 && n_isects >= 0 && tile_w > 0 && tile_h > 0 && (key_bits == 24 || key_bits == 32), "bad sizes or key width");
    GS_CHECK_ARG(n_isects < (1ll << 31), "n_isects must fit int32");
    GS_CHECK_ARG((int64_t)tile_w * tile_h < (1ll << 24) && tile_w < 65536 && tile_h < 65536, "tile grid too large");
    GS_CHECK_ARG(isect_offsets != nullptr && (counts_dev == nullptr || status_dev != nullptr), "null argument");
    hipStream_t s = (hipStream_t)stream;
    const int n_tiles = tile_w * tile_h;
    if (V == 0 || n_isects == 0) { GS_CHECK_HIP(gs_zero_async(isect_offsets, sizeof(int32_t) * (size_t)n_tiles, s)); return GS_OK; }
    GS_CHECK_ARG(depth_keys != nullptr && tile_rects != nullptr && flatten_ids_sorted != nullptr && ws != nullptr, "null argument");
    if (ws_bytes < gs_isect_bin_front_ws_bytes(V, n_isects, tile_w, tile_h)) { gs_set_error("gs_isect_bin_front: workspace too small"); return GS_ENOSPC; }
    const GsCount vc{ (long long)V, (const long long*)counts_dev }, ic{ (long long)n_isects, counts_dev ? (const long long*)counts_dev + 1 : nullptr };
    const bool hist = tile_counts != nullptr && n_tiles <= BF_HIST_MAX;
    char* p = (char*)ws;
    unsigned* table = (unsigned*)p; p += table_bytes((int64_t)V > n_isects ? (int64_t)V : n_isects);
    uint2* da = (uint2*)p; p += align256((size_t)V * 8);
    uint2* db = (uint2*)p; p += align256((size_t)V * 8);
    uint2* ia = (uint2*)p; p += align256((size_t)n_isects * 8);
    uint2* ib = (uint2*)p; p += align256((size_t)n_isects * 8);
    unsigned* state = (unsigned*)p; p += bf_state_bytes(V);
    int32_t* tile_ids = hist ? nullptr : (int32_t*)p;
    const int eblocks = (V + EM_TILE - 1) / EM_TILE;
    const int n_state_words = (int)(bf_state_bytes(V) / 4);
    hipLaunchKernelGGL(bin_setup_kernel, dim3(gs_cdiv(n_state_words, 256) < 64 ? gs_cdiv(n_state_words, 256) : 64),
                       dim3(256), 0, s, state, n_state_words, (const long long*)counts_dev,
                       (long long)V_cap, (long long)n_isects_cap, (long long*)status_dev);
    GS_CHECK_LAUNCH();
    int rc = radix_pass<uint2>(vc, KeyIn{ depth_keys }, XDigit{ 0, 255u }, U2Out{ da }, 8, table, s);
    if (rc != GS_OK) return rc;
    rc = radix_pass<uint2>(vc, U2In{ da }, XDigit{ 8, 255u }, U2Out{ db }, 8, table, s);
    if (rc != GS_OK) return rc;
    rc = radix_pass<uint2>(vc, U2In{ db }, XDigit{ 16, 255u }, U2Out{ da }, 8, table, s);
    if (rc != GS_OK) return rc;
    const uint2* order = da;
    if (key_bits == 32) {
        rc = radix_pass<uint2>(vc, U2In{ da }, XDigit{ 24, 255u }, U2Out{ db }, 8, table, s);
        if (rc != GS_OK) return rc;
        order = db;
    }
    unsigned* ctrl = state; u64* desc = (u64*)((char*)state + 16);
    hipLaunchKernelGGL(emit_chained_kernel, dim3(eblocks), dim3(EM_THREADS), 0, s, vc, order, (const uint2*)tile_rects, ctrl, desc,
                       eblocks + 1, tile_w, ia, (unsigned)n_isects, (long long*)status_dev);
    GS_CHECK_LAUNCH();
    if (hist) {
        hipLaunchKernelGGL(tile_offsets_scan_kernel, dim3(1), dim3(1024), 0, s, n_tiles, (const unsigned*)tile_counts, ic, isect_offsets);
        GS_CHECK_LAUNCH();
    }
    int tb = 0;
    while ((1 << tb) < n_tiles) ++tb;
    if (tb < 1) tb = 1;
    const int npass = (tb + 7) / 8, width = (tb + npass - 1) / npass;
    uint2* src = ia; uint2* dst = ib;
    for (int pass = 0; pass < npass; ++pass) {
        const int shift = pass * width;
        const int nbits = (tb - shift) < width ? (tb - shift) : width;
        if (pass == npass - 1 && hist)
            rc = radix_pass<uint2>(ic, U2In{ src }, XDigit{ shift, (1u << nbits) - 1u }, FinalFlat{ flatten_ids_sorted }, nbits, table, s);
        else if (pass == npass - 1)
            rc = radix_pass<uint2>(ic, U2In{ src }, XDigit{ shift, (1u << nbits) - 1u }, FinalTiles{ tile_ids, flatten_ids_sorted }, nbits, table, s);
        else
            rc = radix_pass<uint2>(ic, U2In{ src }, XDigit{ shift, (1u << nbits) - 1u }, U2Out{ dst }, nbits, table, s);
        if (rc != GS_OK) return rc;
        uint2* t = src; src = dst; dst = t;
    }
    if (!hist) {
        hipLaunchKernelGGL(bin_offsets_tiles_kernel, dim3(gs_cdiv(n_isects, 256)), dim3(256), 0, s, ic, tile_ids, n_tiles, isect_offsets);
        GS_CHECK_LAUNCH();
    }
    return GS_OK;
}

static int isect_bin_impl(int V, const float* means2d, const int32_t* radii, const float* depths, int64_t n_isects,
                          const long long* counts_dev, int tile_size, int tile_w, int tile_h, int64_t* isect_ids_sorted,
                          int32_t* flatten_ids_sorted, void* ws, size_t ws_bytes, void* stream, int32_t* tile_ids_sorted)
{
    const GsCount vc{ (long long)V, counts_dev }, ic{ (long long)n_isects, counts_dev ? counts_dev + 1 : nullptr };
    GS_CHECK_ARG(V >= 0 && n_isects >= 0 && tile_size > 0 && tile_w > 0 && tile_h > 0, "bad sizes");
    GS_CHECK_ARG(n_isects < (1ll << 31), "n_isects must fit int32");
    GS_CHECK_ARG((int64_t)tile_w * tile_h < (1ll << 24), "more than 2^24 tiles");
    if (V == 0 || n_isects == 0) return GS_OK;
    GS_CHECK_ARG(ws != nullptr, "workspace must not be NULL");
    if (ws_bytes < gs_isect_bin_ws_bytes(V, n_isects, tile_w, tile_h)) { gs_set_error("gs_isect_bin: workspace too small"); return GS_ENOSPC; }
    hipStream_t s = (hipStream_t)stream;
    char* p = (char*)ws;
    unsigned* table = (unsigned*)p; p += table_bytes((int64_t)V > n_isects ? (int64_t)V : n_isects);
    uint2* da = (uint2*)p; p += align256((size_t)V * 8);
    uint2* db = (uint2*)p; p += align256((size_t)V * 8);
    uint2* rect = (uint2*)p; p += align256((size_t)V * 8);
    const int eblocks = (V + EM_TILE - 1) / EM_TILE;
    unsigned* state = (unsigned*)p; p += bf_state_bytes(V);
    uint2* ia = (uint2*)p; p += align256((size_t)n_isects * 8);
    uint2* ib = (uint2*)p; p += align256((size_t)n_isects * 8);
    int tb = 0;
    while ((1 << tb) < tile_w * tile_h) ++tb;
    if (tb < 1) tb = 1;
    const int npass = (tb + 7) / 8, width = (tb + npass - 1) / npass;
    int rc = GS_OK;
    rc = radix_pass<uint2>(vc, DepthIn{ depths }, XDigit{ 0, 255u }, U2Out{ da }, 8, table, s);
    if (rc != GS_OK) return rc;
    rc = radix_pass<uint2>(vc, U2In{ da }, XDigit{ 8, 255u }, U2Out{ db }, 8, table, s);
    if (rc != GS_OK) return rc;
    rc = radix_pass<uint2>(vc, U2In{ db }, XDigit{ 16, 255u }, U2Out{ da }, 8, table, s);
    if (rc != GS_OK) return rc;
    rc = radix_pass<uint2>(vc, U2In{ da }, XDigit{ 24, 255u }, U2Out{ db }, 8, table, s);
    if (rc != GS_OK) return rc;
    GS_CHECK_ARG(tile_w < 65536 && tile_h < 65536, "tile grid too large");
    hipLaunchKernelGGL(tile_rect_kernel, dim3(gs_cdiv(V, 256)), dim3(256), 0, s, vc, means2d, radii, tile_size, tile_w, tile_h, rect);
    GS_CHECK_LAUNCH();
    {
        const int n_state_words = (int)(bf_state_bytes(V) / 4);
        hipLaunchKernelGGL(bin_setup_kernel, dim3(gs_cdiv(n_state_words, 256) < 64 ? gs_cdiv(n_state_words, 256) : 64), dim3(256), 0, s, state,
                           n_state_words, (const long long*)nullptr, 0ll, 0ll, (long long*)nullptr);
        GS_CHECK_LAUNCH();
        hipLaunchKernelGGL(emit_chained_kernel, dim3(eblocks), dim3(EM_THREADS), 0, s, vc, (const uint2*)db, (const uint2*)rect, state,
                           (u64*)((char*)state + 16), eblocks + 1, tile_w, ia, (unsigned)n_isects, (long long*)nullptr);
        GS_CHECK_LAUNCH();
    }
    uint2* src = ia; uint2* dst = ib;
    for (int pass = 0; pass < npass; ++pass) {
        const int shift = pass * width;
        const int nbits = (tb - shift) < width ? (tb - shift) : width;
        if (pass == npass - 1 && tile_ids_sorted != nullptr)
            rc = radix_pass<uint2>(ic, U2In{ src }, XDigit{ shift, (1u << nbits) - 1u },
                                   FinalTiles{ tile_ids_sorted, flatten_ids_sorted }, nbits, table, s);
        else if (pass == npass - 1)
            rc = radix_pass<uint2>(ic, U2In{ src }, XDigit{ shift, (1u << nbits) - 1u },
                                   FinalOut{ (u64*)isect_ids_sorted, flatten_ids_sorted, depths }, nbits, table, s);
        else
            rc = radix_pass<uint2>(ic, U2In{ src }, XDigit{ shift, (1u << nbits) - 1u }, U2Out{ dst }, nbits, table, s);
        if (rc != GS_OK) return rc;
        uint2* t = src; src = dst; dst = t;
    }
    return GS_OK;
}
```

geosplatting_amd/front.py:

```python
from __future__ import annotations

import ctypes as C
import os
from typing import Optional

import torch
from torch import Tensor

from . import _lib as L

_pinned_pool4 = []


def pinned_counts4() -> Tensor:
    return _pinned_pool4.pop() if _pinned_pool4 else torch.empty(4, dtype=torch.int64).pin_memory()


def release_counts4(t: Tensor) -> None:
    _pinned_pool4.append(t)


def reserve_pinned(n: int) -> None:
    while len(_pinned_pool4) < n:
        _pinned_pool4.append(torch.empty(4, dtype=torch.int64).pin_memory())


class Front:
    __slots__ = ("vis", "keys", "rects", "tile_counts", "packed_index", "counts", "host_counts", "event", "whs", "key_bits", "N")


def front_stage(means: Tensor, quats: Tensor, scales: Tensor, opacities: Tensor, normals: Tensor, kd: Tensor, ks: Tensor,
                viewmat: Tensor, K: Tensor, cam_pos: Tensor, env_struct, W: int, H: int, min_roughness: float, max_metallic: float,
                mode: int, key_base: int = 0, key_bits: int = 32, status: Optional[Tensor] = None, tile_size: int = 16,
                eps2d: float = 0.3, near: float = 0.01, far: float = 1e10, radius_clip: float = 0.0, want_packed_index: bool = False,
                records: bool = True, binning: bool = True, tight_tiles: bool = False) -> Front:
    lib = L.lib()
    dev = means.device
    N = means.shape[0]
    fr = Front()
    fr.vis = torch.empty(max(N, 1), 16, dtype=torch.float32, device=dev) if records else None
    fr.keys = torch.empty(max(N, 1), dtype=torch.int32, device=dev) if binning else None
    fr.rects = torch.empty(max(N, 1), 2, dtype=torch.int32, device=dev) if binning else None
    fr.counts = torch.empty(4, dtype=torch.int64, device=dev)
    tw, th = (W + tile_size - 1) // tile_size, (H + tile_size - 1) // tile_size
    fr.tile_counts = torch.empty(tw * th, dtype=torch.int32, device=dev) if (binning and tw * th <= 8192) else None
    fr.packed_index = torch.empty(max(N, 1), dtype=torch.int32, device=dev) if want_packed_index else None
    ws_bytes = lib.gs_front_ws_bytes(N)
    ws = torch.empty(ws_bytes, dtype=torch.uint8, device=dev)
    L.check(lib.gs_front_fwd(N, L.ptr(means), L.ptr(quats), L.ptr(scales), L.ptr(opacities), L.ptr(normals), L.ptr(kd), L.ptr(ks),
                             L.ptr(viewmat), L.ptr(K), L.ptr(cam_pos), L.f32(min_roughness), L.f32(max_metallic), mode,
                             C.byref(env_struct) if env_struct is not None else None, W, H, tile_size, L.f32(eps2d), L.f32(near), L.f32(far), L.f32(radius_clip),
                             C.c_uint32(int(key_base) & 0xffffffff), int(key_bits), L.ptr(fr.vis), L.ptr(fr.keys), L.ptr(fr.rects),
                             L.ptr(fr.tile_counts), L.ptr(fr.packed_index), 1 if tight_tiles else 0, L.ptr(fr.counts), L.ptr(status), L.ptr(ws), C.c_size_t(ws_bytes), L.stream()), "gs_front_fwd")
    fr.host_counts = pinned_counts4()
    fr.host_counts.copy_(fr.counts, non_blocking=True)
    fr.event = torch.cuda.Event()
    fr.event.record()
    fr.whs = (W, H, tile_size)
    fr.key_bits = int(key_bits)
    fr.N = N
    return fr


def depth_range(host_counts: Tensor):
    if int(host_counts[0]) <= 0:
        return None
    return 0xffffffff - int(host_counts[2]), int(host_counts[3])


def learn_depth_range(lo: Optional[int], hi: Optional[int], host_counts: Tensor):
    rng = depth_range(host_counts)
    if rng is None:
        return lo, hi
    return (rng[0] if lo is None else min(lo, rng[0])), (rng[1] if hi is None else max(hi, rng[1]))


def binning_keys(lo: Optional[int], hi: Optional[int]):
    if lo is None:
        return 32, 0
    base = max(0, lo - (1 << 22))
    if hi - base < (1 << 24) - (1 << 21):
        return 24, base
    return 32, 0


def bin_stage(fr: Front, i_cap: Optional[int], status: Optional[Tensor], prepare: bool = True, binned=None):
    lib = L.lib()
    W, H, tile_size = fr.whs
    dev = fr.counts.device
    tw, th = (W + tile_size - 1) // tile_size, (H + tile_size - 1) // tile_size
    st = L.stream()
    if i_cap is None:
        fr.event.synchronize()
        V, I = int(fr.host_counts[0]), int(fr.host_counts[1])
        if V < 0 or I < 0 or I >= 2 ** 31:
            raise L.GeoSplatHipError(f"bad intersection count V={V} I={I}")
        counts = None
    else:
        V, I, counts = fr.N, int(i_cap), fr.counts
    if binned is not None:
        flat, offsets = binned
    else:
        flat = torch.empty(max(I, 1), dtype=torch.int32, device=dev)
        offsets = torch.empty(th * tw, dtype=torch.int32, device=dev)
        bin_bytes = lib.gs_isect_bin_front_ws_bytes(V, L.i64(I), tw, th)
        bin_ws = torch.empty(max(bin_bytes, 1), dtype=torch.uint8, device=dev)
        L.check(lib.gs_isect_bin_front(V, L.ptr(fr.keys), L.ptr(fr.rects), L.ptr(fr.tile_counts), L.ptr(counts), L.i64(I), fr.key_bits, tw, th,
                                       L.ptr(flat), L.ptr(offsets), L.ptr(bin_ws), C.c_size_t(bin_bytes),
                                       L.ptr(status) if counts is not None else None, st), "gs_isect_bin_front")
    if not prepare:
        return dict(flatten_ids=flat, isect_offsets=offsets, counts=counts, keys=fr.keys, rects=fr.rects, tile_counts=fr.tile_counts), V, I
    rws_bytes = lib.gs_raster_ws_bytes(L.i64(I), V, W, H, tile_size)
    rws = torch.empty(rws_bytes, dtype=torch.uint8, device=dev)
    if counts is None:
        L.check(lib.gs_raster_prepare_vis(W, H, tile_size, 3, V, L.ptr(fr.vis), L.i64(I), L.ptr(offsets), L.ptr(flat), L.ptr(rws),
                                          C.c_size_t(rws_bytes), st), "gs_raster_prepare_vis")
    else:
        L.check(lib.gs_raster_prepare_vis_cap(W, H, tile_size, 3, V, L.ptr(fr.vis), L.i64(I), L.ptr(counts), L.ptr(offsets), L.ptr(flat),
                                              L.ptr(rws), C.c_size_t(rws_bytes), st), "gs_raster_prepare_vis_cap")
    state = dict(vis_records=fr.vis, flatten_ids=flat, isect_offsets=offsets, raster_ws=rws, counts=counts, keys=fr.keys, rects=fr.rects,
                 tile_counts=fr.tile_counts, packed_index=fr.packed_index)
    return state, V, I


def tail_stage(V: int, counts: Optional[Tensor], means: Tensor, quats: Tensor, scales: Tensor, opacities: Tensor, normals: Tensor,
               kd: Tensor, ks: Tensor, viewmat: Tensor, K: Tensor, cam_pos: Tensor, env_struct, env_grad_struct, W: int, H: int,
               min_roughness: float, max_metallic: float, mode: int, vis: Tensor, v_packed: Tensor, g_means: Tensor, g_quats: Tensor,
               g_scales: Tensor, g_opacities: Tensor, g_normals: Tensor, g_kd: Tensor, g_ks: Tensor, eps2d: float = 0.3,
               priv: Optional[Tensor] = None) -> None:
    lib = L.lib()
    L.check(lib.gs_tail_bwd(V, L.ptr(counts), L.ptr(means), L.ptr(quats), L.ptr(scales), L.ptr(opacities), L.ptr(normals), L.ptr(kd),
                            L.ptr(ks), L.ptr(viewmat), L.ptr(K), L.ptr(cam_pos), L.f32(min_roughness), L.f32(max_metallic), mode,
                            C.byref(env_struct), W, H, L.f32(eps2d), L.ptr(vis), L.ptr(v_packed), int(v_packed.shape[1]),
                            L.ptr(g_means), L.ptr(g_quats), L.ptr(g_scales), L.ptr(g_opacities), L.ptr(g_normals), L.ptr(g_kd),
                            L.ptr(g_ks), C.byref(env_grad_struct), L.ptr(priv), C.c_size_t(0 if priv is None else priv.numel()),
                            L.stream()), "gs_tail_bwd")


def tail_priv_alloc(env_struct, mode: int, device) -> Optional[Tensor]:
    n = L.lib().gs_tail_priv_ws_bytes(C.byref(env_struct), mode)
    return torch.zeros(n, dtype=torch.uint8, device=device) if n > 0 else None


def tail_priv_reduce(env_struct, env_grad_struct, mode: int, priv: Optional[Tensor]) -> None:
    if priv is not None:
        L.check(L.lib().gs_tail_priv_reduce(C.byref(env_struct), mode, L.ptr(priv), C.c_size_t(priv.numel()), C.byref(env_grad_struct),
                                            L.stream()), "gs_tail_priv_reduce")


def tail_multi_stage(views, means: Tensor, quats: Tensor, scales: Tensor, opacities: Tensor, normals: Tensor, kd: Tensor, ks: Tensor,
                     env_struct, env_grad_struct, min_roughness: float, max_metallic: float, mode: int, g_means: Tensor, g_quats: Tensor,
                     g_scales: Tensor, g_opacities: Tensor, g_normals: Tensor, g_kd: Tensor, g_ks: Tensor, accumulate: bool,
                     eps2d: float = 0.3, priv: Optional[Tensor] = None, parts: int = 3) -> None:
    lib = L.lib()
    arr = (L.GsTailView * len(views))()
    stride = None
    for i, (vm, K, cp, vis, vp, pidx, W, H) in enumerate(views):
        arr[i].viewmat = vm.data_ptr(); arr[i].K = K.data_ptr(); arr[i].cam_pos = cp.data_ptr()
        arr[i].vis_records = vis.data_ptr(); arr[i].v_packed = vp.data_ptr(); arr[i].packed_index = pidx.data_ptr()
        arr[i].W = int(W); arr[i].H = int(H)
        assert stride in (None, int(vp.shape[1]))
        stride = int(vp.shape[1])
    L.check(lib.gs_tail_bwd_multi_parts(int(parts), means.shape[0], len(views), arr, L.ptr(means), L.ptr(quats), L.ptr(scales), L.ptr(opacities), L.ptr(normals),
                                  L.ptr(kd), L.ptr(ks), L.f32(min_roughness), L.f32(max_metallic), mode, C.byref(env_struct), L.f32(eps2d),
                                  stride, L.ptr(g_means), L.ptr(g_quats), L.ptr(g_scales), L.ptr(g_opacities), L.ptr(g_normals), L.ptr(g_kd),
                                  L.ptr(g_ks), 1 if accumulate else 0, C.byref(env_grad_struct), L.ptr(priv),
                                  C.c_size_t(0 if priv is None else priv.numel()), L.stream()), "gs_tail_bwd_multi_parts")


def front_streams(dev: torch.device):
    return [L.shared_stream(dev, "front0"), L.shared_stream(dev, "front1")]


class CameraCache:
    MAX_ENTRIES = 4096

    def __init__(self, dev: torch.device):
        self.dev = dev
        self.entries = {}

    def get(self, cam, stream: torch.cuda.Stream):
        c2w = cam.c2w
        intr = (float(cam.fx), float(cam.fy), float(cam.cx), float(cam.cy), int(cam.width), int(cam.height))
        host = c2w.device.type == "cpu"
        fp = c2w.detach().numpy().tobytes() if host else None
        key = (c2w.data_ptr(), tuple(c2w.shape), tuple(c2w.stride()), intr)
        hit = self.entries.get(key)
        if hit is not None and hit[1] == c2w._version and hit[3] == fp:
            return hit[2]
        if len(self.entries) >= self.MAX_ENTRIES:
            self.entries.pop(next(iter(self.entries)))
        caller = torch.cuda.current_stream(self.dev)
        if not host and stream != caller:
            stream.wait_stream(caller)
        with torch.cuda.stream(stream):
            tensors = (cam.view_matrix.to(self.dev, torch.float32).contiguous(),
                       cam.intrinsic_matrix.to(self.dev, torch.float32).contiguous(),
                       c2w.detach()[:, 3].to(self.dev, torch.float32).contiguous())
            ev = torch.cuda.Event(); ev.record(stream)
        for f in front_streams(self.dev):
            if f != stream:
                f.wait_event(ev)
        self.entries[key] = (c2w, c2w._version, tensors, fp)
        return tensors

    def clear(self) -> None:
        self.entries.clear()


def texel_grads(env, flat: Optional[Tensor] = None):
    sizes = [env.base.numel()] + [l.numel() for l in env.levels]
    if flat is None or flat.numel() != sum(sizes):
        flat = torch.zeros(sum(sizes), dtype=torch.float32, device=env.base.device)
    parts = torch.split(flat, sizes)
    g_base = parts[0].view_as(env.base)
    g_levels = [q.view_as(l) for q, l in zip(parts[1:], env.levels)]
    eg = L.GsEnvGrad(); eg.base = g_base.data_ptr()
    for i, g in enumerate(g_levels):
        eg.levels[i] = g.data_ptr()
    return flat, g_base, g_levels, eg


def log_ws(I: int, W: int, H: int, dev: torch.device) -> Tensor:
    return torch.empty(L.lib().gs_raster_log_ws_bytes(L.i64(I), W, H, 16), dtype=torch.uint8, device=dev)


def composite_fwd(state, V: int, I: int, W: int, H: int, tone: int, exposure: Tensor, log: Tensor):
    dev = state["isect_offsets"].device
    f32 = torch.float32
    render = torch.empty(H, W, 3, dtype=f32, device=dev); alphas = torch.empty(H, W, dtype=f32, device=dev)
    last_ids = torch.empty(H, W, dtype=torch.int32, device=dev); img = torch.empty(H, W, 4, dtype=f32, device=dev)
    rws = state["raster_ws"]
    L.check(L.lib().gs_raster_composite_tone_log(W, H, 16, V, None, L.i64(I), L.ptr(state["counts"]), L.ptr(state["isect_offsets"]),
                                                 L.ptr(render), L.ptr(alphas), L.ptr(last_ids), tone, L.ptr(exposure), L.ptr(img),
                                                 L.ptr(rws), C.c_size_t(rws.numel()), L.ptr(log), C.c_size_t(log.numel()), L.stream()),
            "gs_raster_composite_tone_log")
    return img, render, alphas, last_ids


def composite_bwd(state, V: int, I: int, W: int, H: int, tone: int, exposure: Tensor, render: Tensor, alphas: Tensor,
                  last_ids: Tensor, log: Tensor, v_img: Tensor, g_exp: Tensor) -> None:
    rws = state["raster_ws"]
    L.check(L.lib().gs_raster_bwd_tone_log_acc(W, H, 16, V, None, L.i64(I), L.ptr(state["counts"]), L.ptr(state["isect_offsets"]),
                                               L.ptr(render), L.ptr(alphas), L.ptr(last_ids), tone, L.ptr(exposure), L.ptr(v_img),
                                               L.ptr(state["v_packed"]), L.ptr(g_exp), L.ptr(rws), C.c_size_t(rws.numel()), L.ptr(log),
                                               C.c_size_t(log.numel()), L.stream()), "gs_raster_bwd_tone_log_acc")


def tail_schedule(default):
    tb = os.environ.get("GEOSPLAT_TAIL_BATCH", "auto")
    return default if tb == "auto" else [max(1, int(x)) for x in tb.split(",")]


def tail_batch(views, args, accumulate: bool, final: bool, tail: torch.cuda.Stream, proj: torch.cuda.Stream, tail_events=None):
    timed = final and tail_events is not None
    ev = torch.cuda.Event(); ev.record(torch.cuda.current_stream(tail.device))
    tail.wait_event(ev)
    with torch.cuda.stream(tail):
        if timed:
            t0 = torch.cuda.Event(enable_timing=True); t0.record(tail)
        tail_multi_stage(views, *args, accumulate=accumulate, parts=1 if final else 7)
    used = [tail]
    if final:
        ev_sh = torch.cuda.Event(enable_timing=timed); ev_sh.record(tail)
        proj.wait_event(ev_sh)
        with torch.cuda.stream(proj):
            tail_multi_stage(views, *args, accumulate=accumulate, parts=2)
            if timed:
                t2 = torch.cuda.Event(enable_timing=True); t2.record(proj)
                tail_events.append((t0, ev_sh, t2))
        used.append(proj)
    for v in views:
        for t in v[:6]:
            for s in used:
                t.record_stream(s)
    return used


def status_overflow(word: Tensor):
    w = word.tolist()
    return w[0] != 0 or w[3] != 0, w[3] != 0, w[1]
```

include/geosplat_hip.h:

```cpp
#ifndef GEOSPLAT_HIP_H
#define GEOSPLAT_HIP_H

#include <stddef.h>
#include <stdint.h>

#ifdef __cplusplus
extern "C" {
#endif

#define GS_OK            0
#define GS_EINVAL       -1
#define GS_ENOSPC       -2
#define GS_ELAUNCH      -3

#define GS_MAX_LEVELS   16
#define GS_MAX_CHANNELS 32

#define GS_MODE_PBR      0
#define GS_MODE_DIFFUSE  1
#define GS_MODE_SPECULAR 2
#define GS_TONE_NONE     0
#define GS_TONE_NAIVE    1
#define GS_TONE_ACES     2

const char* gs_last_error(void);
int         gs_version(void);

size_t gs_project_ws_bytes(int N);

int gs_project_fwd(int N, const float* means, const float* quats, const float* scales, const float* opacities,
                   const float* colors, int D, const float* viewmat, const float* K, int W, int H, int tile_size,
                   float eps2d, float near_plane, float far_plane, float radius_clip,
                   int32_t* gaussian_ids, int32_t* radii, float* means2d, float* depths, float* conics,
                   float* compensations, float* opacities_packed, float* colors_packed,
                   int32_t* tiles_per_gauss, int64_t* cum_tiles, int32_t* packed_index,
                   void* ws, size_t ws_bytes, int64_t* counts, void* stream);

int gs_project_fwd_vis(int N, const float* means, const float* quats, const float* scales, const float* opacities,
                       const float* colors, int D, const float* viewmat, const float* K, int W, int H, int tile_size,
                       float eps2d, float near_plane, float far_plane, float radius_clip,
                       int32_t* gaussian_ids, int32_t* radii, float* means2d, float* depths, float* conics,
                       float* compensations, float* opacities_packed, float* colors_packed,
                       int32_t* tiles_per_gauss, int64_t* cum_tiles, int32_t* packed_index, float* vis_records,
                       void* ws, size_t ws_bytes, int64_t* counts, void* stream);

#define GS_PROJ_CLASSIC 1
int gs_project_fwd_vis_ex(int N, const float* means, const float* quats, const float* scales, const float* opacities,
                          const float* colors, int D, const float* sh_coeffs, int sh_K, int sh_degree, int flags,
                          const float* viewmat, const float* K, int W, int H, int tile_size,
                          float eps2d, float near_plane, float far_plane, float radius_clip,
                          int32_t* gaussian_ids, int32_t* radii, float* means2d, float* depths, float* conics,
                          float* compensations, float* opacities_packed, float* colors_packed,
                          int32_t* tiles_per_gauss, int64_t* cum_tiles, int32_t* packed_index, float* vis_records,
                          void* ws, size_t ws_bytes, int64_t* counts, void* stream);

int gs_isect_emit(int V, const float* means2d, const int32_t* radii, const float* depths,
                  const int64_t* cum_tiles, int tile_size, int tile_w, int tile_h,
                  int64_t* isect_ids, int32_t* flatten_ids, void* stream);

size_t gs_isect_bin_ws_bytes(int V, int64_t n_isects, int tile_w, int tile_h);
int gs_isect_bin(int V, const float* means2d, const int32_t* radii, const float* depths, const int32_t* tiles_per_gauss,
                 int64_t n_isects, int tile_size, int tile_w, int tile_h, int64_t* isect_ids_sorted,
                 int32_t* flatten_ids_sorted, void* ws, size_t ws_bytes, void* stream);

size_t gs_sort_ws_bytes(int64_t n_isects, int tile_w, int tile_h);
int gs_isect_sort(int64_t n_isects, const int64_t* isect_ids, const int32_t* flatten_ids,
                  int64_t* isect_ids_sorted, int32_t* flatten_ids_sorted, int tile_w, int tile_h,
                  void* ws, size_t ws_bytes, void* stream);

int gs_isect_offsets(int64_t n_isects, const int64_t* isect_ids_sorted, int n_tiles, int32_t* offsets,
                     void* stream);

size_t gs_raster_ws_bytes(int64_t n_isects, int V, int W, int H, int tile_size);

int gs_raster_fwd(int W, int H, int tile_size, int D, int V, const float* means2d, const float* conics,
                  const float* opacities, const float* colors, const float* background,
                  int64_t n_isects, const int32_t* offsets, const int32_t* flatten_ids,
                  float* render, float* alphas, int32_t* last_ids, void* ws, size_t ws_bytes, void* stream);

int gs_raster_prepare(int W, int H, int tile_size, int D, int V, const float* means2d, const float* conics,
                      const float* opacities, const float* colors, int64_t n_isects, const int32_t* offsets,
                      const int32_t* flatten_ids, void* ws, size_t ws_bytes, void* stream);
int gs_raster_prepare_vis(int W, int H, int tile_size, int D, int V, const float* vis_records ,
                          int64_t n_isects, const int32_t* offsets, const int32_t* flatten_ids, void* ws, size_t ws_bytes,
                          void* stream);
int gs_raster_composite(int W, int H, int tile_size, int D, int V, const float* colors, const float* background,
                        int64_t n_isects, const int32_t* offsets, float* render, float* alphas, int32_t* last_ids,
                        const void* ws, size_t ws_bytes, void* stream);

int gs_raster_grad_stride(int D);

int gs_raster_bwd(int W, int H, int tile_size, int D, int V, const float* colors, const float* background,
                  int64_t n_isects, const int32_t* offsets, const float* alphas, const int32_t* last_ids,
                  const float* v_render, const float* v_alphas, float* v_packed, const void* ws, size_t ws_bytes,
                  void* stream);

int gs_raster_bwd_acc(int W, int H, int tile_size, int D, int V, const float* colors, const float* background,
                      int64_t n_isects, const int32_t* offsets, const float* alphas, const int32_t* last_ids,
                      const float* v_render, const float* v_alphas, float* v_packed, const void* ws, size_t ws_bytes,
                      void* stream);

int gs_isect_bin_cap(int V_cap, const float* means2d, const int32_t* radii, const float* depths, const int64_t* counts_dev,
                     int64_t n_isects_cap, int tile_size, int tile_w, int tile_h, int64_t* isect_ids_sorted,
                     int32_t* flatten_ids_sorted, void* ws, size_t ws_bytes, int64_t* status_dev, void* stream);
int gs_isect_offsets_cap(int64_t n_isects_cap, const int64_t* counts_dev, const int64_t* isect_ids_sorted, int n_tiles,
                         int32_t* offsets, void* stream);
int gs_isect_bin_tiles_cap(int V_cap, const float* means2d, const int32_t* radii, const float* depths, const int64_t* counts_dev,
                           int64_t n_isects_cap, int tile_size, int tile_w, int tile_h, int32_t* tile_ids_sorted,
                           int32_t* flatten_ids_sorted, void* ws, size_t ws_bytes, int64_t* status_dev, void* stream);
int gs_isect_offsets_tiles_cap(int64_t n_isects_cap, const int64_t* counts_dev, const int32_t* tile_ids_sorted, int n_tiles,
                               int32_t* offsets, void* stream);
int gs_raster_prepare_vis_cap(int W, int H, int tile_size, int D, int V_cap, const float* vis_records, int64_t n_isects_cap,
                              const int64_t* counts_dev, const int32_t* offsets, const int32_t* flatten_ids, void* ws,
                              size_t ws_bytes, void* stream);
int gs_raster_composite_cap(int W, int H, int tile_size, int D, int V_cap, const float* colors, const float* background,
                            int64_t n_isects_cap, const int64_t* counts_dev, const int32_t* offsets, float* render,
                            float* alphas, int32_t* last_ids, const void* ws, size_t ws_bytes, void* stream);
int gs_raster_bwd_cap(int W, int H, int tile_size, int D, int V_cap, const float* colors, const float* background,
                      int64_t n_isects_cap, const int64_t* counts_dev, const int32_t* offsets, const float* alphas,
                      const int32_t* last_ids, const float* v_render, const float* v_alphas, float* v_packed, const void* ws,
                      size_t ws_bytes, void* stream);
int gs_raster_bwd_acc_cap(int W, int H, int tile_size, int D, int V_cap, const float* colors, const float* background,
                          int64_t n_isects_cap, const int64_t* counts_dev, const int32_t* offsets, const float* alphas,
                          const int32_t* last_ids, const float* v_render, const float* v_alphas, float* v_packed, const void* ws,
                          size_t ws_bytes, void* stream);
int gs_raster_composite_tone(int W, int H, int tile_size, int V, const float* colors, int64_t n_isects,
                             const int64_t* counts_dev, const int32_t* offsets, float* render, float* alphas,
                             int32_t* last_ids, int tone_mode, const float* exposure , float* image,
                             const void* ws, size_t ws_bytes, void* stream);
int gs_raster_bwd_tone_acc(int W, int H, int tile_size, int V, const float* colors, int64_t n_isects,
                           const int64_t* counts_dev, const int32_t* offsets, const float* render, const float* alphas,
                           const int32_t* last_ids, int tone_mode, const float* exposure, const float* v_image,
                           float* v_packed, float* v_exposure, const void* ws, size_t ws_bytes, void* stream);
size_t gs_raster_log_ws_bytes(int64_t n_isects, int W, int H, int tile_size);
int gs_raster_composite_tone_log(int W, int H, int tile_size, int V, const float* colors, int64_t n_isects,
                                 const int64_t* counts_dev, const int32_t* offsets, float* render, float* alphas,
                                 int32_t* last_ids, int tone_mode, const float* exposure, float* image, const void* ws,
                                 size_t ws_bytes, void* log_ws, size_t log_bytes, void* stream);
int gs_raster_bwd_tone_log_acc(int W, int H, int tile_size, int V, const float* colors, int64_t n_isects,
                               const int64_t* counts_dev, const int32_t* offsets, const float* render, const float* alphas,
                               const int32_t* last_ids, int tone_mode, const float* exposure, const float* v_image,
                               float* v_packed, float* v_exposure, const void* ws, size_t ws_bytes, const void* log_ws,
                               size_t log_bytes, void* stream);
int gs_project_bwd_cap(int N, const int64_t* counts_dev, int D, const float* means, const float* quats, const float* scales,
                       const float* opacities, const float* viewmat, const float* K, int W, int H, float eps2d,
                       const int32_t* gaussian_ids, const float* conics, const float* compensations, const float* v_packed,
                       int rec_stride, const float* v_depths, float* v_means, float* v_quats, float* v_scales,
                       float* v_opacities, float* v_colors, int accumulate, void* stream);

int gs_selftest_rcp(uint32_t lo_bits, uint32_t hi_bits, uint64_t* mismatches_dev, void* stream);

int gs_selftest_exp(uint32_t lo_bits, uint32_t hi_bits, uint64_t* out_dev, void* stream);

int gs_selftest_cube_edges(int R, uint64_t* mismatches_dev, void* stream);

int gs_project_bwd(int N, int V, int D, const float* means, const float* quats, const float* scales,
                   const float* opacities, const float* viewmat, const float* K, int W, int H, float eps2d,
                   const int32_t* gaussian_ids, const float* conics, const float* compensations,
                   const float* v_packed, int rec_stride , const float* v_depths,
                   float* v_means, float* v_quats, float* v_scales, float* v_opacities, float* v_colors,
                   int accumulate, void* stream);

int gs_project_bwd_ex(int N, int V, int D, const float* means, const float* quats, const float* scales,
                      const float* opacities, const float* viewmat, const float* K, int W, int H, float eps2d,
                      const int32_t* gaussian_ids, const float* conics, const float* compensations,
                      const float* v_packed, int rec_stride, const float* v_depths, const float* sh_coeffs, int sh_K,
                      int sh_degree, int flags, float* v_means, float* v_quats, float* v_scales, float* v_opacities,
                      float* v_colors, float* g_sh_coeffs, int accumulate, void* stream);

typedef struct GsEnv {
    const float* lut;
    int          lut_res;
    const float* base;
    int          base_res;
    int          num_levels;
    const float* levels[GS_MAX_LEVELS];
    int          res[GS_MAX_LEVELS];
    float        min_roughness;
    float        max_roughness;
} GsEnv;

typedef struct GsEnvGrad {
    float* base;
    float* levels[GS_MAX_LEVELS];
} GsEnvGrad;

int gs_shade_fwd(int N, const float* means, const float* normals, const float* kd, const float* ks,
                 const float* cam_pos, float min_roughness, float max_metallic, int mode,
                 const GsEnv* env , float* colors, void* stream);

size_t gs_shade_bwd_ws_bytes(const GsEnv* env , int mode);

int gs_shade_bwd(int N, const float* means, const float* normals, const float* kd, const float* ks,
                 const float* cam_pos, float min_roughness, float max_metallic, int mode,
                 const GsEnv* env , const float* v_colors,
                 float* v_means, float* v_normals, float* v_kd, float* v_ks,
                 const GsEnvGrad* env_grad , int accumulate, void* ws, size_t ws_bytes, void* stream);

int gs_tonemap_fwd(int64_t P, int mode, const float* rgba, const float* exposure, float* out, void* stream);
int gs_tonemap_fwd3(int64_t P, int mode, const float* render, const float* alphas, const float* exposure, float* out, void* stream);
int gs_tonemap_bwd3(int64_t P, int mode, const float* render, const float* alphas, const float* exposure, const float* v_out,
                    float* v_render, float* v_alphas, float* v_exposure, int accumulate, void* stream);
int gs_tonemap_bwd(int64_t P, int mode, const float* rgba, const float* exposure, const float* v_out,
                   float* v_rgba, float* v_exposure, int accumulate, void* stream);

int gs_cubemap_mip_fwd(int R, int C, const float* in, float* out, void* stream);
int gs_cubemap_mip_chain_fwd(int R, int n_levels, const float* in, float* const* outs, void* stream);
int gs_cube_sample_linear(int64_t n, const float* tex, int R, const float* dirs, float scale, float* out,
                          void* stream);
int gs_cubemap_mip_bwd(int R, const float* v_out, float* v_in, int accumulate, void* stream);
int gs_diffuse_cubemap_fwd(int R, const float* cubemap, float* out, void* stream);
int gs_diffuse_cubemap_bwd(int R, const float* v_out, float* v_cubemap, int accumulate, void* stream);
int gs_specular_bounds(int R, float costheta_cutoff, float* bounds, void* stream);
size_t gs_specular_bounds_ws_bytes(int R);
int gs_specular_bounds_fast(int R, float costheta_cutoff, const float* dir_table, float* bounds, void* ws, size_t ws_bytes, void* stream);
int gs_cube_dir_table(int R, float* table, void* stream);
int gs_specular_cubemap_fwd(int R, const float* cubemap, const float* bounds, const float* dir_table,
                            float roughness, float costheta_cutoff, float* out, void* stream);
int gs_specular_cubemap_bwd(int R, const float* bounds, const float* dir_table, const float* v_out_rgb,
                            float roughness, float costheta_cutoff, float* v_cubemap, int accumulate, void* stream);

int gs_specular_tiles_count(int R, float roughness, float costheta_cutoff, int backward, int margin, int bw, int nb, const float* bounds,
                            const float* dir_table, const int32_t* tiles, int n_tiles, int32_t* row_counts, int32_t* extents,
                            uint64_t* pairs, void* stream);
int gs_specular_tiles_fill(int R, float roughness, float costheta_cutoff, int backward, int margin, int bw, int nb, const float* bounds,
                           const float* dir_table, const int32_t* tiles, int n_tiles, const int64_t* row_begin,
                           const int32_t* segments, int32_t* desc, float* weights, void* stream);
int gs_specular_tiles_check(int R, const float* bounds, const float* dir_table, uint64_t* out2, void* stream);
int gs_specular_tiles_apply(int R, int backward, int n_mirrors, int margin, int bw, int nb, const float* src, const float* scale,
                            const float* out_scale, const float* bounds, const int32_t* tiles, const int32_t* segments,
                            const int64_t* row_begin, const int32_t* row_counts, const int32_t* desc, const float* weights, float* dst,
                            int tile_begin, int tile_end, size_t lds_bytes, void* stream);

typedef struct GsTileLevel {
    int R, n_mirrors, margin, bw, nb, tile_begin, tile_end, reserved;
    const float* src; const float* scale; const float* out_scale; const float* bounds;
    const int32_t* tiles; const int32_t* segments; const int64_t* row_begin; const int32_t* row_counts; const int32_t* desc;
    const float* weights; float* dst; size_t lds_bytes;
} GsTileLevel;
int gs_specular_tiles_apply_multi(int n_levels, const GsTileLevel* levels, int backward, void* stream);

int gs_mgadapter_fwd(int F, const float* vertices, const int64_t* faces, const float* vnormals,
                     float* means, float* scales, float* quats, float* normals, void* stream);
int gs_mgadapter_bwd(int F, int V, const float* vertices, const int64_t* faces, const float* vnormals,
                     const float* v_means, const float* v_scales, const float* v_quats, const float* v_normals,
                     float* v_vertices, float* v_vnormals, void* stream);

int gs_vertex_normals_fwd(int F, int V, const float* vertices, const int64_t* faces, float* raw, float* vnormals,
                          void* stream);
int gs_vertex_normals_bwd(int F, int V, const float* vertices, const int64_t* faces, const float* raw,
                          const float* v_vnormals, float* v_raw, float* v_vertices, int accumulate, void* stream);

size_t gs_photo_loss_ws_bytes(int W, int H);
int gs_photo_loss(int W, int H, const float* rgb, const float* alpha, const float* gt_rgba, int gt_is_srgb,
                  const float* train_bg, const float* metric_bg, float ssim_lambda, float mask_weight,
                  float grad_scale, float* out, float* v_rgb, float* v_alpha, void* ws, size_t ws_bytes, void* stream);

int gs_hashgrid_fwd(int N, int L, int F, int log2_T, const float* scalings_host, const float* x, const float* table,
                    float* out, void* stream);
size_t gs_hashgrid_bwd_ws_bytes(int N, int L, int F);
int gs_hashgrid_bwd(int N, int L, int F, int log2_T, const float* scalings_host, const float* x, const float* table,
                    const float* v_out, float table_grad_scale, float* v_table, int accumulate, float* v_x,
                    void* ws ,
                    size_t ws_bytes, void* stream);

size_t gs_hashgrid_bwd_fixed_ws_bytes(int N, int L, int F, int log2_T);
int gs_hashgrid_bwd_fixed(int N, int L, int F, int log2_T, const float* scalings_host, const float* x, const float* table,
                          const float* v_out, float table_grad_scale, float* v_table, int accumulate, float* v_x, void* ws,
                          size_t ws_bytes, void* stream);

size_t gs_mlp_wgrad_ws_bytes(int64_t N);
int gs_mlp_wgrad(int64_t N, int O, int I, const float* dY, const float* X, float scale, float* dW, int accumulate,
                 void* ws, size_t ws_bytes, void* stream);

size_t gs_flexicubes_ws_bytes(int R0, int R1, int R2);
int gs_flexicubes_count(int R0, int R1, int R2, const float* sdf, void* ws, size_t ws_bytes, int64_t* counts, void* stream);
int gs_flexicubes_fwd(int R0, int R1, int R2, const float* vertices, const float* sdf, const float* alpha,
                      const float* beta, const float* gamma, float weight_scale, float sdf_eps, const void* ws,
                      size_t ws_bytes, int64_t Q, int64_t num_quads, int64_t K, float* out_vertices, int64_t* out_faces,
                      float* L_dev, void* stream);
int gs_flexicubes_bwd(int R0, int R1, int R2, const float* vertices, const float* sdf, const float* alpha,
                      const float* beta, const float* gamma, float weight_scale, float sdf_eps, const void* ws,
                      size_t ws_bytes, int64_t Q, int64_t num_quads, int64_t K, const float* out_vertices,
                      const float* v_out_vertices, const float* v_L_dev, float* g_vd_scratch, float* g_vertices,
                      float* g_sdf, float* g_alpha, float* g_beta, float* g_gamma, void* stream);
int gs_flexicubes_entropy_fwd(int R0, int R1, int R2, const float* sdf, void* ws, size_t ws_bytes, float* out, void* stream);
int gs_flexicubes_entropy_bwd(int R0, int R1, int R2, const float* sdf, const void* ws, size_t ws_bytes, const float* v_out,
                              float* g_sdf, int accumulate, void* stream);

size_t gs_front_ws_bytes(int N);
int gs_front_fwd(int N, const float* means, const float* quats, const float* scales, const float* opacities,
                 const float* normals, const float* kd, const float* ks, const float* viewmat, const float* K,
                 const float* cam_pos, float min_roughness, float max_metallic, int mode, const GsEnv* env,
                 int W, int H, int tile_size, float eps2d, float near_plane, float far_plane, float radius_clip,
                 uint32_t key_base, int key_bits, float* vis_records, uint32_t* depth_keys, uint32_t* tile_rects,
                 uint32_t* tile_counts, int32_t* packed_index ,
                 int tight_tiles, int64_t* counts4, int64_t* status4, void* ws, size_t ws_bytes, void* stream);
size_t gs_isect_bin_front_ws_bytes(int V, int64_t n_isects, int tile_w, int tile_h);
int gs_isect_bin_front(int V_cap, const uint32_t* depth_keys, const uint32_t* tile_rects, const uint32_t* tile_counts,
                       const int64_t* counts_dev, int64_t n_isects_cap, int key_bits, int tile_w, int tile_h, int32_t* flatten_ids_sorted,
                       int32_t* isect_offsets, void* ws, size_t ws_bytes, int64_t* status_dev, void* stream);
int gs_tail_bwd(int V_cap, const int64_t* counts_dev, const float* means, const float* quats, const float* scales,
                const float* opacities, const float* normals, const float* kd, const float* ks, const float* viewmat,
                const float* K, const float* cam_pos, float min_roughness, float max_metallic, int mode, const GsEnv* env,
                int W, int H, float eps2d, const float* vis_records, const float* v_packed, int rec_stride,
                float* v_means, float* v_quats, float* v_scales, float* v_opacities, float* v_normals, float* v_kd, float* v_ks,
                const GsEnvGrad* env_grad, void* priv_ws, size_t priv_ws_bytes, void* stream);
typedef struct GsTailView {
    const float* viewmat; const float* K; const float* cam_pos;
    const float* vis_records; const float* v_packed; const int32_t* packed_index;
    int W, H;
} GsTailView;
int gs_tail_bwd_multi(int N, int n_views, const GsTailView* views , const float* means, const float* quats,
                      const float* scales, const float* opacities, const float* normals, const float* kd, const float* ks,
                      float min_roughness, float max_metallic, int mode, const GsEnv* env, float eps2d, int rec_stride,
                      float* v_means, float* v_quats, float* v_scales, float* v_opacities, float* v_normals, float* v_kd, float* v_ks,
                      int accumulate, const GsEnvGrad* env_grad, void* priv_ws, size_t priv_ws_bytes, void* stream);
int gs_tail_bwd_multi_parts(int parts, int N, int n_views, const GsTailView* views , const float* means, const float* quats,
                            const float* scales, const float* opacities, const float* normals, const float* kd, const float* ks,
                            float min_roughness, float max_metallic, int mode, const GsEnv* env, float eps2d, int rec_stride,
                            float* v_means, float* v_quats, float* v_scales, float* v_opacities, float* v_normals, float* v_kd, float* v_ks,
                            int accumulate, const GsEnvGrad* env_grad, void* priv_ws, size_t priv_ws_bytes, void* stream);
size_t gs_tail_priv_ws_bytes(const GsEnv* env , int mode);
int gs_tail_priv_reduce(const GsEnv* env , int mode, const void* priv_ws, size_t priv_ws_bytes, const GsEnvGrad* env_grad,
                        void* stream);

int gs_activation_chain(int64_t N, const float* g_scales_act, const float* scales_act, const float* g_opac_act, const float* opac_act,
                        float* v_scales, float* v_opacities, void* stream);

#ifdef __cplusplus
}
#endif
#endif
```

Baseline: 714.3.

## Fuse record gathering into final bin sort and carry rects through depth sort

The depth radix sort now carries each Gaussian's tile rect alongside its key, so emit reads rects sequentially instead of gathering them. Emit also builds the first tile-sort pass histogram with LDS atomics, which removes one histogram kernel. A new streaming bin path writes the raster records (rec0/1/2) directly from the final sort scatter, and a separate order-only prepare skips the record-packing pass. This trades extra sort traffic (wider items, two-phase staging) and global atomics for fewer kernels and less rereading of intersections.

```diff
diff --git a/geosplatting_amd/_lib.py b/geosplatting_amd/_lib.py
--- a/geosplatting_amd/_lib.py
+++ b/geosplatting_amd/_lib.py
@@ -43,7 +43,7 @@
     "gs_specular_tiles_check", "gs_specular_tiles_apply", "gs_specular_tiles_apply_multi", "gs_mgadapter_fwd", "gs_mgadapter_bwd", "gs_vertex_normals_fwd",
     "gs_vertex_normals_bwd", "gs_photo_loss_ws_bytes", "gs_photo_loss", "gs_hashgrid_fwd", "gs_hashgrid_bwd_ws_bytes", "gs_hashgrid_bwd", "gs_hashgrid_bwd_fixed_ws_bytes", "gs_hashgrid_bwd_fixed", "gs_mlp_wgrad_ws_bytes", "gs_mlp_wgrad",
     "gs_flexicubes_ws_bytes", "gs_flexicubes_count", "gs_flexicubes_fwd", "gs_flexicubes_bwd", "gs_flexicubes_entropy_fwd",
-    "gs_flexicubes_entropy_bwd", "gs_front_ws_bytes", "gs_front_fwd", "gs_isect_bin_front_ws_bytes", "gs_isect_bin_front", "gs_tail_bwd", "gs_tail_bwd_multi", "gs_tail_bwd_multi_parts", "gs_tail_priv_ws_bytes", "gs_tail_priv_reduce", "gs_activation_chain",
+    "gs_flexicubes_entropy_bwd", "gs_front_ws_bytes", "gs_front_fwd", "gs_isect_bin_front_ws_bytes", "gs_isect_bin_front", "gs_isect_bin_front_stream", "gs_raster_prepare_order", "gs_tail_bwd", "gs_tail_bwd_multi", "gs_tail_bwd_multi_parts", "gs_tail_priv_ws_bytes", "gs_tail_priv_reduce", "gs_activation_chain",
 ]
 
 _lib: Optional[C.CDLL] = None
diff --git a/geosplatting_amd/csrc/gs_common.h b/geosplatting_amd/csrc/gs_common.h
--- a/geosplatting_amd/csrc/gs_common.h
+++ b/geosplatting_amd/csrc/gs_common.h
@@ -42,6 +42,19 @@
 {
     for (size_t i = (size_t)blockIdx.x * blockDim.x + threadIdx.x; i < n_words; i += (size_t)gridDim.x * blockDim.x) p[i] = 0u;
 }
+struct GsRecords { float4 *rec0, *rec1, *rec2; };
+static inline size_t gs_records_seg_bytes(int64_t n_isects)
+{
+    const size_t n = n_isects > 0 ? (size_t)n_isects : 1;
+    return (n * sizeof(float4) + 255) & ~(size_t)255;
+}
+static inline GsRecords gs_raster_records(void* ws, int64_t n_isects)
+{
+    char* p = (char*)ws;
+    const size_t seg = gs_records_seg_bytes(n_isects);
+    return GsRecords{ (float4*)p, (float4*)(p + seg), (float4*)(p + 2 * seg) };
+}
+
 static __global__ void __launch_bounds__(256) gs_zero16_kernel(uint4* __restrict__ p, size_t n_quads)
 {
     for (size_t i = (size_t)blockIdx.x * blockDim.x + threadIdx.x; i < n_quads; i += (size_t)gridDim.x * blockDim.x) p[i] = make_uint4(0u, 0u, 0u, 0u);
diff --git a/geosplatting_amd/csrc/gs_raster.hip b/geosplatting_amd/csrc/gs_raster.hip
--- a/geosplatting_amd/csrc/gs_raster.hip
+++ b/geosplatting_amd/csrc/gs_raster.hip
@@ -1390,11 +1390,10 @@
 {
     const size_t n = n_isects > 0 ? (size_t)n_isects : 1;
     const size_t v = V > 0 ? (size_t)V : 1;
-    char* p = (char*)ws;
+    const GsRecords rec = gs_raster_records(ws, n_isects);
+    char* p = (char*)ws + 3 * gs_records_seg_bytes(n_isects);
     RasterWs r;
-    r.rec0 = (float4*)p; p += align256(n * sizeof(float4));
-    r.rec1 = (float4*)p; p += align256(n * sizeof(float4));
-    r.rec2 = (float4*)p; p += align256(n * sizeof(float4));
+    r.rec0 = rec.rec0; r.rec1 = rec.rec1; r.rec2 = rec.rec2;
     r.order = (int32_t*)p; p += align256((size_t)tiles * sizeof(int32_t));
     r.bo.bcount = (int32_t*)p; p += align256(64 * sizeof(int32_t));
     r.bo.blist = (int32_t*)p; p += align256(64 * (size_t)tiles * sizeof(int32_t));
@@ -1452,14 +1451,14 @@
 static int raster_prepare_impl(int W, int H, int tile_size, int D, int V, const float* means2d, const float* conics,
                                const float* opacities, const float* colors, const float* vis_records, int64_t n_isects,
                                const int32_t* offsets, const int32_t* flatten_ids, void* ws, size_t ws_bytes, void* stream,
-                               const RasterOpts& o)
+                               const RasterOpts& o, bool build_stream = true)
 {
     const int rc = raster_check("gs_raster_prepare", W, H, tile_size, D, V, n_isects, ws, ws_bytes);
     if (rc != GS_OK) return rc;
     hipStream_t s = (hipStream_t)stream;
     const int tiles = ((W + GS_TILE - 1) / GS_TILE) * ((H + GS_TILE - 1) / GS_TILE);
     const RasterWs r = carve(ws, n_isects, V, tiles);
-    if (n_isects > 0 && V > 0) {
+    if (build_stream && n_isects > 0 && V > 0) {
         const float4* vis = (const float4*)vis_records;
         if (!vis) {
             hipLaunchKernelGGL(pack_visible_kernel, dim3(gs_cdiv(V, 256)), dim3(256), 0, s, V, D, means2d, conics, opacities, colors,
@@ -1586,6 +1585,15 @@
                                flatten_ids, ws, ws_bytes, stream, RasterOpts{});
 }
 
+extern "C" int gs_raster_prepare_order(int W, int H, int tile_size, int D, int V, int64_t n_isects, const int64_t* counts_dev,
+                                       const int32_t* offsets, void* ws, size_t ws_bytes, void* stream)
+{
+    RasterOpts o;
+    o.counts = counts_dev;
+    return raster_prepare_impl(W, H, tile_size, D, V, nullptr, nullptr, nullptr, nullptr, nullptr, n_isects, offsets, nullptr, ws,
+                               ws_bytes, stream, o, false);
+}
+
 extern "C" int gs_raster_composite(int W, int H, int tile_size, int D, int V, const float* colors, const float* background,
                                    int64_t n_isects, const int32_t* offsets, float* render, float* alphas,
                                    int32_t* last_ids, const void* ws, size_t ws_bytes, void* stream)
diff --git a/geosplatting_amd/csrc/gs_sort.hip b/geosplatting_amd/csrc/gs_sort.hip
--- a/geosplatting_amd/csrc/gs_sort.hip
+++ b/geosplatting_amd/csrc/gs_sort.hip
@@ -2,6 +2,7 @@
 
 #include <cstdlib>
 #include <cstring>
+#include <type_traits>
 
 #define RS_THREADS 256
 #define RS_WAVES 4
@@ -41,13 +42,30 @@
     uint2* p;
     __device__ __forceinline__ void store(int64_t i, const uint2& it) const { p[i] = it; }
 };
-struct DepthIn {
-    const float* depths;
-    __device__ __forceinline__ uint2 load(int64_t i) const { return make_uint2(__float_as_uint(depths[i]), (unsigned)i); }
+struct DepthRectIn {
+    const float* depths; const uint2* rects;
+    __device__ __forceinline__ uint4 load(int64_t i) const
+    {
+        const uint2 q = rects[i];
+        return make_uint4(__float_as_uint(depths[i]), (unsigned)i, q.x, q.y);
+    }
 };
 struct XDigit {
     int shift; unsigned mask;
     __device__ __forceinline__ unsigned operator()(const uint2& it) const { return (it.x >> shift) & mask; }
+    __device__ __forceinline__ unsigned operator()(const uint4& it) const { return (it.x >> shift) & mask; }
+};
+struct U4In {
+    const uint2* kv; const uint2* rc;
+    __device__ __forceinline__ uint4 load(int64_t i) const { const uint2 a = kv[i], b = rc[i]; return make_uint4(a.x, a.y, b.x, b.y); }
+};
+struct U4Out {
+    uint2* kv; uint2* rc;
+    __device__ __forceinline__ void store_half(int64_t i, int h, const uint2& v) const { (h ? rc : kv)[i] = v; }
+};
+struct OrderOut {
+    unsigned* idx; uint2* rc;
+    __device__ __forceinline__ void store_half(int64_t i, int h, const uint2& v) const { if (h) rc[i] = v; else idx[i] = v.y; }
 };
 struct FinalTiles {
     int32_t* tile_ids; int32_t* flatten_ids;
@@ -114,10 +132,12 @@
 {
     const int64_t n = gs_count(nc);
     constexpr int NB = 1 << NBITS;
+    constexpr bool WIDE = std::is_same<Item, uint4>::value;
+    using Stage = typename std::conditional<WIDE, uint2, Item>::type;
     __shared__ unsigned cnt[RS_WAVES][NB];
     __shared__ unsigned dstart[NB];
     __shared__ unsigned gbase[NB];
-    __shared__ Item stage[RS_TILE];
+    __shared__ Stage stage[RS_TILE];
     const int lane = threadIdx.x & 63, wave = threadIdx.x >> 6;
     for (int i = threadIdx.x; i < RS_WAVES * NB; i += RS_THREADS) (&cnt[0][0])[i] = 0u;
     __syncthreads();
@@ -175,37 +195,66 @@
         if (d < NB) gbase[d] = rbefore + rincl - rt + table[(size_t)d * nblocks + blockIdx.x];
     }
     __syncthreads();
+    unsigned slot[RS_ITEMS];
 #pragma unroll
     for (int k = 0; k < RS_ITEMS; ++k) {
         const int64_t i = wbase + (int64_t)k * 64 + lane;
+        slot[k] = 0u;
         if (i < n) {
             const unsigned d = dig[k];
             unsigned off = dstart[d] + rank[k];
             for (int w = 0; w < wave; ++w) off += cnt[w][d];
-            stage[off] = item[k];
+            slot[k] = off;
+            if constexpr (WIDE) stage[off] = make_uint2(item[k].x, item[k].y);
+            else stage[off] = item[k];
         }
     }
     __syncthreads();
+    if constexpr (WIDE) {
+        int64_t dst[RS_ITEMS];
+#pragma unroll
+        for (int k = 0; k < RS_ITEMS; ++k) {
+            const int p = k * RS_THREADS + (int)threadIdx.x;
+            dst[k] = 0;
+            if (p < n_here) {
+                const uint2 it = stage[p];
+                const unsigned d = digit(it);
+                dst[k] = (int64_t)gbase[d] + (int64_t)(p - (int)dstart[d]);
+                out.store_half(dst[k], 0, it);
+            }
+        }
+        __syncthreads();
+#pragma unroll
+        for (int k = 0; k < RS_ITEMS; ++k) {
+            const int64_t i = wbase + (int64_t)k * 64 + lane;
+            if (i < n) stage[slot[k]] = make_uint2(item[k].z, item[k].w);
+        }
+        __syncthreads();
+#pragma unroll
+        for (int k = 0; k < RS_ITEMS; ++k) {
+            const int p = k * RS_THREADS + (int)threadIdx.x;
+            if (p < n_here) out.store_half(dst[k], 1, stage[p]);
+        }
+    } else {
 #pragma unroll 4
-    for (int k = 0; k < RS_ITEMS; ++k) {
-        const int p = k * RS_THREADS + (int)threadIdx.x;
-        if (p < n_here) {
-            const Item it = stage[p];
-            const unsigned d = digit(it);
-            out.store((int64_t)gbase[d] + (int64_t)(p - (int)dstart[d]), it);
+        for (int k = 0; k < RS_ITEMS; ++k) {
+            const int p = k * RS_THREADS + (int)threadIdx.x;
+            if (p < n_here) {
+                const Item it = stage[p];
+                const unsigned d = digit(it);
+                out.store((int64_t)gbase[d] + (int64_t)(p - (int)dstart[d]), it);
+            }
         }
     }
 }
 
 template <typename Item, typename In, typename Digit, typename Out>
-static int radix_pass(GsCount nc, In in, Digit digit, Out out, int nbits, unsigned* table, hipStream_t s)
+static int radix_pass_counted(GsCount nc, In in, Digit digit, Out out, int nbits, unsigned* table, hipStream_t s)
 {
     const int64_t n = nc.n;
     const int nblocks = (int)((n + RS_TILE - 1) / RS_TILE);
     const int nbins = 1 << nbits;
     unsigned* row_total = table + (size_t)256 * nblocks;
-    hipLaunchKernelGGL((radix_hist_kernel<Item, In, Digit>), dim3(nblocks), dim3(RS_THREADS), 0, s, nc, in, digit, nbins, nblocks, table);
-    GS_CHECK_LAUNCH();
     hipLaunchKernelGGL(radix_rowscan_kernel, dim3(nbins), dim3(256), 0, s, nblocks, table, row_total);
     GS_CHECK_LAUNCH();
     switch (nbits) {
@@ -216,6 +265,15 @@
     }
     GS_CHECK_LAUNCH();
     return GS_OK;
+}
+
+template <typename Item, typename In, typename Digit, typename Out>
+static int radix_pass(GsCount nc, In in, Digit digit, Out out, int nbits, unsigned* table, hipStream_t s)
+{
+    const int nblocks = (int)((nc.n + RS_TILE - 1) / RS_TILE);
+    hipLaunchKernelGGL((radix_hist_kernel<Item, In, Digit>), dim3(nblocks), dim3(RS_THREADS), 0, s, nc, in, digit, 1 << nbits, nblocks, table);
+    GS_CHECK_LAUNCH();
+    return radix_pass_counted<Item>(nc, in, digit, out, nbits, table, s);
 }
 
 static size_t align256(size_t x) { return (x + 255) & ~(size_t)255; }
@@ -303,7 +361,7 @@
     (void)tile_w; (void)tile_h;
     const size_t v = V > 0 ? (size_t)V : 1, n = n_isects > 0 ? (size_t)n_isects : 1;
     const size_t tb = table_bytes((int64_t)(v > n ? v : n));
-    return tb + 3 * align256(v * 8) + bf_state_bytes((int)v) + 2 * align256(n * 8) + 256;
+    return tb + table_bytes((int64_t)n) + 5 * align256(v * 8) + bf_state_bytes((int)v) + 2 * align256(n * 8) + 256;
 }
 
 __global__ void capacity_check_kernel(const long long* __restrict__ counts, long long v_cap, long long i_cap, long long* __restrict__ status)
@@ -354,23 +412,38 @@
                           nullptr, flatten_ids_sorted, ws, ws_bytes, stream, tile_ids_sorted);
 }
 
-struct KeyIn {
-    const unsigned* keys;
-    __device__ __forceinline__ uint2 load(int64_t i) const { return make_uint2(keys[i], (unsigned)i); }
+struct KeyRectIn {
+    const unsigned* keys; const uint2* rects;
+    __device__ __forceinline__ uint4 load(int64_t i) const { const uint2 q = rects[i]; return make_uint4(keys[i], (unsigned)i, q.x, q.y); }
 };
 struct FinalFlat {
     int32_t* flatten_ids;
     __device__ __forceinline__ void store(int64_t i, const uint2& it) const { flatten_ids[i] = (int32_t)it.y; }
 };
+struct FinalStream {
+    int32_t* flatten_ids; int32_t* tile_ids; const float4* vis; GsRecords rec;
+    __device__ __forceinline__ void store(int64_t i, const uint2& it) const
+    {
+        const int g = (int)it.y;
+        flatten_ids[i] = g;
+        if (tile_ids) tile_ids[i] = (int32_t)it.x;
+        const float4* v = vis + 4 * (size_t)g;
+        const float4 a = v[0], b = v[1];
+        float4 c = v[2];
+        c.w = __int_as_float(g);
+        rec.rec0[i] = a; rec.rec1[i] = b; rec.rec2[i] = c;
+    }
+};
 
 #define BF_HIST_MAX 8192
 
 __global__ void __launch_bounds__(256)
-bin_setup_kernel(unsigned* __restrict__ state, int n_state_words,
+bin_setup_kernel(unsigned* __restrict__ state, int n_state_words, unsigned* __restrict__ ttable, int n_ttable_words,
                  const long long* __restrict__ counts, long long v_cap, long long i_cap, long long* __restrict__ status)
 {
     const int i = blockIdx.x * blockDim.x + threadIdx.x, stride = gridDim.x * blockDim.x;
     for (int k = i; k < n_state_words; k += stride) state[k] = 0u;
+    for (int k = i; k < n_ttable_words; k += stride) ttable[k] = 0u;
     if (i == 0 && counts != nullptr && status != nullptr) {
         const long long V = counts[0], I = counts[1];
         if (V > v_cap || I > i_cap) {
@@ -384,17 +457,25 @@
 #define BF_VALID (1ull << 63)
 #define BF_SPIN_LIMIT (1 << 22)
 
+#define EM_HSLOTS 4
+
+struct TileHist {
+    unsigned* table; int nblocks; unsigned mask; GsCount nc;
+};
+
 __global__ void __launch_bounds__(EM_THREADS)
-emit_chained_kernel(GsCount vc, const uint2* __restrict__ order, const uint2* __restrict__ rect, unsigned* __restrict__ ctrl,
-                    u64* __restrict__ desc, int n_blocks, int tile_w, uint2* __restrict__ items, unsigned item_cap,
+emit_chained_kernel(GsCount vc, const unsigned* __restrict__ idx, const uint2* __restrict__ rect, unsigned* __restrict__ ctrl,
+                    u64* __restrict__ desc, int n_blocks, int tile_w, uint2* __restrict__ items, unsigned item_cap, TileHist th,
                     long long* __restrict__ status )
 {
     const int V = (int)gs_count(vc);
     __shared__ unsigned ws[EM_THREADS / 64];
     __shared__ unsigned s_block;
     __shared__ unsigned long long s_base;
+    __shared__ unsigned hist[EM_HSLOTS][256];
     const int lane = threadIdx.x & 63, wave = threadIdx.x >> 6;
     if (threadIdx.x == 0) s_block = atomicAdd(ctrl, 1u);
+    for (int i = threadIdx.x; i < EM_HSLOTS * 256; i += EM_THREADS) (&hist[0][0])[i] = 0u;
     __syncthreads();
     const int block = (int)s_block;
     u64* agg = desc; u64* pre = desc + n_blocks;
@@ -404,8 +485,8 @@
 #pragma unroll
     for (int k = 0; k < EM_PER; ++k) {
         const int r = r0 + k;
-        v[k] = r < V ? (int)order[r].y : -1;
-        q[k] = v[k] >= 0 ? rect[v[k]] : make_uint2(0u, 0u);
+        v[k] = r < V ? (int)idx[r] : -1;
+        q[k] = r < V ? rect[r] : make_uint2(0u, 0u);
         c[k] = rect_count(q[k]);
         mine += c[k];
     }
@@ -464,6 +545,8 @@
         }
     }
     __syncthreads();
+    const unsigned long long n_hist = (unsigned long long)gs_count(th.nc);
+    const unsigned long long rb0 = s_base / RS_TILE;
     unsigned long long cur = s_base + before + incl - mine;
 #pragma unroll
     for (int k = 0; k < EM_PER; ++k) {
@@ -473,10 +556,22 @@
             for (int j = x0; j < x1; ++j) {
                 const unsigned t = (unsigned)(i * tile_w + j);
                 if (cur < (unsigned long long)item_cap) items[cur] = make_uint2(t, (unsigned)v[k]);
+                if (cur < n_hist) {
+                    const unsigned long long rb = cur / RS_TILE;
+                    if (rb - rb0 < EM_HSLOTS) atomicAdd(&hist[rb - rb0][t & th.mask], 1u);
+                    else atomicAdd(&th.table[(size_t)(t & th.mask) * th.nblocks + rb], 1u);
+                }
                 ++cur;
             }
     }
-}
+    __syncthreads();
+    for (int i = threadIdx.x; i < EM_HSLOTS * 256; i += EM_THREADS) {
+        const unsigned h = (&hist[0][0])[i];
+        const unsigned long long rb = rb0 + (unsigned)(i / 256);
+        if (h != 0u) atomicAdd(&th.table[(size_t)(i % 256) * th.nblocks + rb], h);
+    }
+}
+
 
 __global__ void __launch_bounds__(1024)
 tile_offsets_scan_kernel(int n_tiles, const unsigned* __restrict__ tile_counts, GsCount nc, int32_t* __restrict__ offsets)
@@ -524,12 +619,13 @@
 {
     const size_t v = V > 0 ? (size_t)V : 1, n = n_isects > 0 ? (size_t)n_isects : 1;
     const size_t tb = table_bytes((int64_t)(v > n ? v : n));
-    return tb + 2 * align256(v * 8) + 2 * align256(n * 8) + bf_state_bytes((int)v) + align256(n * 4) + 256;
-}
-
-extern "C" int gs_isect_bin_front(int V_cap, const uint32_t* depth_keys, const uint32_t* tile_rects, const uint32_t* tile_counts,
-                                  const int64_t* counts_dev, int64_t n_isects_cap, int key_bits, int tile_w, int tile_h, int32_t* flatten_ids_sorted,
-                                  int32_t* isect_offsets, void* ws, size_t ws_bytes, int64_t* status_dev, void* stream)
+    return tb + table_bytes((int64_t)n) + 4 * align256(v * 8) + 2 * align256(n * 8) + bf_state_bytes((int)v) + align256(n * 4) + 256;
+}
+
+static int isect_bin_front_impl(int V_cap, const uint32_t* depth_keys, const uint32_t* tile_rects, const uint32_t* tile_counts,
+                                const int64_t* counts_dev, int64_t n_isects_cap, int key_bits, int tile_w, int tile_h, int32_t* flatten_ids_sorted,
+                                int32_t* isect_offsets, void* ws, size_t ws_bytes, int64_t* status_dev, void* stream, const float4* vis,
+                                const GsRecords* rec)
 {
     const int V = V_cap;
     const int64_t n_isects = n_isects_cap;
@@ -546,52 +642,70 @@
     const bool hist = tile_counts != nullptr && n_tiles <= BF_HIST_MAX;
     char* p = (char*)ws;
     unsigned* table = (unsigned*)p; p += table_bytes((int64_t)V > n_isects ? (int64_t)V : n_isects);
+    unsigned* ttable = (unsigned*)p; p += table_bytes(n_isects);
     uint2* da = (uint2*)p; p += align256((size_t)V * 8);
     uint2* db = (uint2*)p; p += align256((size_t)V * 8);
+    uint2* ra = (uint2*)p; p += align256((size_t)V * 8);
+    uint2* rb = (uint2*)p; p += align256((size_t)V * 8);
     uint2* ia = (uint2*)p; p += align256((size_t)n_isects * 8);
     uint2* ib = (uint2*)p; p += align256((size_t)n_isects * 8);
     unsigned* state = (unsigned*)p; p += bf_state_bytes(V);
     int32_t* tile_ids = hist ? nullptr : (int32_t*)p;
     const int eblocks = (V + EM_TILE - 1) / EM_TILE;
     const int n_state_words = (int)(bf_state_bytes(V) / 4);
-    hipLaunchKernelGGL(bin_setup_kernel, dim3(gs_cdiv(n_state_words, 256) < 64 ? gs_cdiv(n_state_words, 256) : 64),
-                       dim3(256), 0, s, state, n_state_words, (const long long*)counts_dev,
-                       (long long)V_cap, (long long)n_isects_cap, (long long*)status_dev);
-    GS_CHECK_LAUNCH();
-    int rc = radix_pass<uint2>(vc, KeyIn{ depth_keys }, XDigit{ 0, 255u }, U2Out{ da }, 8, table, s);
-    if (rc != GS_OK) return rc;
-    rc = radix_pass<uint2>(vc, U2In{ da }, XDigit{ 8, 255u }, U2Out{ db }, 8, table, s);
-    if (rc != GS_OK) return rc;
-    rc = radix_pass<uint2>(vc, U2In{ db }, XDigit{ 16, 255u }, U2Out{ da }, 8, table, s);
-    if (rc != GS_OK) return rc;
-    const uint2* order = da;
-    if (key_bits == 32) {
-        rc = radix_pass<uint2>(vc, U2In{ da }, XDigit{ 24, 255u }, U2Out{ db }, 8, table, s);
-        if (rc != GS_OK) return rc;
-        order = db;
-    }
-    unsigned* ctrl = state; u64* desc = (u64*)((char*)state + 16);
-    hipLaunchKernelGGL(emit_chained_kernel, dim3(eblocks), dim3(EM_THREADS), 0, s, vc, order, (const uint2*)tile_rects, ctrl, desc,
-                       eblocks + 1, tile_w, ia, (unsigned)n_isects, (long long*)status_dev);
-    GS_CHECK_LAUNCH();
-    if (hist) {
-        hipLaunchKernelGGL(tile_offsets_scan_kernel, dim3(1), dim3(1024), 0, s, n_tiles, (const unsigned*)tile_counts, ic, isect_offsets);
-        GS_CHECK_LAUNCH();
-    }
     int tb = 0;
     while ((1 << tb) < n_tiles) ++tb;
     if (tb < 1) tb = 1;
     const int npass = (tb + 7) / 8, width = (tb + npass - 1) / npass;
+    const int nbits0 = tb < width ? tb : width;
+    const int tnblocks = (int)((n_isects + RS_TILE - 1) / RS_TILE);
+    const int n_ttable_words = (1 << nbits0) * tnblocks;
+    const int setup_blocks = gs_cdiv(n_state_words > n_ttable_words ? n_state_words : n_ttable_words, 256);
+    hipLaunchKernelGGL(bin_setup_kernel, dim3(setup_blocks < 256 ? setup_blocks : 256), dim3(256), 0, s, state, n_state_words, ttable,
+                       n_ttable_words, (const long long*)counts_dev, (long long)V_cap, (long long)n_isects_cap, (long long*)status_dev);
+    GS_CHECK_LAUNCH();
+    const int ndpass = key_bits / 8;
+    uint2* kv[2] = { da, db };
+    uint2* rcs[2] = { ra, rb };
+    int rc = GS_OK;
+    for (int pass = 0; pass < ndpass; ++pass) {
+        const XDigit dg{ pass * 8, 255u };
+        const int o = pass & 1, i = o ^ 1;
+        if (pass == 0)
+            rc = radix_pass<uint4>(vc, KeyRectIn{ depth_keys, (const uint2*)tile_rects }, dg, U4Out{ kv[o], rcs[o] }, 8, table, s);
+        else if (pass < ndpass - 1)
+            rc = radix_pass<uint4>(vc, U4In{ kv[i], rcs[i] }, dg, U4Out{ kv[o], rcs[o] }, 8, table, s);
+        else
+            rc = radix_pass<uint4>(vc, U4In{ kv[i], rcs[i] }, dg, OrderOut{ (unsigned*)kv[o], rcs[o] }, 8, table, s);
+        if (rc != GS_OK) return rc;
+    }
+    const unsigned* order_idx = (const unsigned*)kv[(ndpass - 1) & 1];
+    const uint2* order_rect = rcs[(ndpass - 1) & 1];
+    unsigned* ctrl = state; u64* desc = (u64*)((char*)state + 16);
+    hipLaunchKernelGGL(emit_chained_kernel, dim3(eblocks), dim3(EM_THREADS), 0, s, vc, order_idx, order_rect, ctrl, desc,
+                       eblocks + 1, tile_w, ia, (unsigned)n_isects, TileHist{ ttable, tnblocks, (1u << nbits0) - 1u, ic }, (long long*)status_dev);
+    GS_CHECK_LAUNCH();
+    if (hist) {
+        hipLaunchKernelGGL(tile_offsets_scan_kernel, dim3(1), dim3(1024), 0, s, n_tiles, (const unsigned*)tile_counts, ic, isect_offsets);
+        GS_CHECK_LAUNCH();
+    }
     uint2* src = ia; uint2* dst = ib;
     for (int pass = 0; pass < npass; ++pass) {
         const int shift = pass * width;
         const int nbits = (tb - shift) < width ? (tb - shift) : width;
-        if (pass == npass - 1 && hist)
-            rc = radix_pass<uint2>(ic, U2In{ src }, XDigit{ shift, (1u << nbits) - 1u }, FinalFlat{ flatten_ids_sorted }, nbits, table, s);
+        const XDigit dg{ shift, (1u << nbits) - 1u };
+        auto tile_pass = [&](auto out) {
+            return pass == 0 ? radix_pass_counted<uint2>(ic, U2In{ src }, dg, out, nbits, ttable, s)
+                             : radix_pass<uint2>(ic, U2In{ src }, dg, out, nbits, table, s);
+        };
+        if (pass == npass - 1 && rec != nullptr)
+            rc = tile_pass(FinalStream{ flatten_ids_sorted, tile_ids, vis, *rec });
+        else if (pass == npass - 1 && hist)
+            rc = tile_pass(FinalFlat{ flatten_ids_sorted });
         else if (pass == npass - 1)
-            rc = radix_pass<uint2>(ic, U2In{ src }, XDigit{ shift, (1u << nbits) - 1u }, FinalTiles{ tile_ids, flatten_ids_sorted }, nbits, table, s);
+            rc = tile_pass(FinalTiles{ tile_ids, flatten_ids_sorted });
         else
-            rc = radix_pass<uint2>(ic, U2In{ src }, XDigit{ shift, (1u << nbits) - 1u }, U2Out{ dst }, nbits, table, s);
+            rc = tile_pass(U2Out{ dst });
         if (rc != GS_OK) return rc;
         uint2* t = src; src = dst; dst = t;
     }
@@ -600,6 +714,26 @@
         GS_CHECK_LAUNCH();
     }
     return GS_OK;
+}
+
+extern "C" int gs_isect_bin_front(int V_cap, const uint32_t* depth_keys, const uint32_t* tile_rects, const uint32_t* tile_counts,
+                                  const int64_t* counts_dev, int64_t n_isects_cap, int key_bits, int tile_w, int tile_h, int32_t* flatten_ids_sorted,
+                                  int32_t* isect_offsets, void* ws, size_t ws_bytes, int64_t* status_dev, void* stream)
+{
+    return isect_bin_front_impl(V_cap, depth_keys, tile_rects, tile_counts, counts_dev, n_isects_cap, key_bits, tile_w, tile_h, flatten_ids_sorted,
+                                isect_offsets, ws, ws_bytes, status_dev, stream, nullptr, nullptr);
+}
+
+extern "C" int gs_isect_bin_front_stream(int V_cap, const uint32_t* depth_keys, const uint32_t* tile_rects, const uint32_t* tile_counts,
+                                         const int64_t* counts_dev, int64_t n_isects_cap, int key_bits, int tile_w, int tile_h, const float* vis_records,
+                                         int32_t* flatten_ids_sorted, int32_t* isect_offsets, void* ws, size_t ws_bytes, void* raster_ws,
+                                         size_t raster_ws_bytes, int64_t* status_dev, void* stream)
+{
+    GS_CHECK_ARG(raster_ws != nullptr && (vis_records != nullptr || V_cap == 0), "raster_ws / vis_records must not be NULL");
+    if (raster_ws_bytes < 3 * gs_records_seg_bytes(n_isects_cap)) { gs_set_error("gs_isect_bin_front_stream: raster workspace too small"); return GS_ENOSPC; }
+    const GsRecords rec = gs_raster_records(raster_ws, n_isects_cap);
+    return isect_bin_front_impl(V_cap, depth_keys, tile_rects, tile_counts, counts_dev, n_isects_cap, key_bits, tile_w, tile_h, flatten_ids_sorted,
+                                isect_offsets, ws, ws_bytes, status_dev, stream, (const float4*)vis_records, &rec);
 }
 
 static int isect_bin_impl(int V, const float* means2d, const int32_t* radii, const float* depths, int64_t n_isects,
@@ -613,11 +747,15 @@
     if (V == 0 || n_isects == 0) return GS_OK;
     GS_CHECK_ARG(ws != nullptr, "workspace must not be NULL");
     if (ws_bytes < gs_isect_bin_ws_bytes(V, n_isects, tile_w, tile_h)) { gs_set_error("gs_isect_bin: workspace too small"); return GS_ENOSPC; }
+    GS_CHECK_ARG(tile_w < 65536 && tile_h < 65536, "tile grid too large");
     hipStream_t s = (hipStream_t)stream;
     char* p = (char*)ws;
     unsigned* table = (unsigned*)p; p += table_bytes((int64_t)V > n_isects ? (int64_t)V : n_isects);
+    unsigned* ttable = (unsigned*)p; p += table_bytes(n_isects);
     uint2* da = (uint2*)p; p += align256((size_t)V * 8);
     uint2* db = (uint2*)p; p += align256((size_t)V * 8);
+    uint2* ra = (uint2*)p; p += align256((size_t)V * 8);
+    uint2* rb = (uint2*)p; p += align256((size_t)V * 8);
     uint2* rect = (uint2*)p; p += align256((size_t)V * 8);
     const int eblocks = (V + EM_TILE - 1) / EM_TILE;
     unsigned* state = (unsigned*)p; p += bf_state_bytes(V);
@@ -627,39 +765,44 @@
     while ((1 << tb) < tile_w * tile_h) ++tb;
     if (tb < 1) tb = 1;
     const int npass = (tb + 7) / 8, width = (tb + npass - 1) / npass;
+    const int nbits0 = tb < width ? tb : width;
+    const int tnblocks = (int)((n_isects + RS_TILE - 1) / RS_TILE);
+    const int n_ttable_words = (1 << nbits0) * tnblocks;
+    const int n_state_words = (int)(bf_state_bytes(V) / 4);
     int rc = GS_OK;
-    rc = radix_pass<uint2>(vc, DepthIn{ depths }, XDigit{ 0, 255u }, U2Out{ da }, 8, table, s);
+    hipLaunchKernelGGL(tile_rect_kernel, dim3(gs_cdiv(V, 256)), dim3(256), 0, s, vc, means2d, radii, tile_size, tile_w, tile_h, rect);
+    GS_CHECK_LAUNCH();
+    const int setup_blocks = gs_cdiv(n_state_words > n_ttable_words ? n_state_words : n_ttable_words, 256);
+    hipLaunchKernelGGL(bin_setup_kernel, dim3(setup_blocks < 256 ? setup_blocks : 256), dim3(256), 0, s, state, n_state_words, ttable,
+                       n_ttable_words, (const long long*)nullptr, 0ll, 0ll, (long long*)nullptr);
+    GS_CHECK_LAUNCH();
+    rc = radix_pass<uint4>(vc, DepthRectIn{ depths, rect }, XDigit{ 0, 255u }, U4Out{ da, ra }, 8, table, s);
     if (rc != GS_OK) return rc;
-    rc = radix_pass<uint2>(vc, U2In{ da }, XDigit{ 8, 255u }, U2Out{ db }, 8, table, s);
+    rc = radix_pass<uint4>(vc, U4In{ da, ra }, XDigit{ 8, 255u }, U4Out{ db, rb }, 8, table, s);
     if (rc != GS_OK) return rc;
-    rc = radix_pass<uint2>(vc, U2In{ db }, XDigit{ 16, 255u }, U2Out{ da }, 8, table, s);
+    rc = radix_pass<uint4>(vc, U4In{ db, rb }, XDigit{ 16, 255u }, U4Out{ da, ra }, 8, table, s);
     if (rc != GS_OK) return rc;
-    rc = radix_pass<uint2>(vc, U2In{ da }, XDigit{ 24, 255u }, U2Out{ db }, 8, table, s);
+    rc = radix_pass<uint4>(vc, U4In{ da, ra }, XDigit{ 24, 255u }, OrderOut{ (unsigned*)db, rb }, 8, table, s);
     if (rc != GS_OK) return rc;
-    GS_CHECK_ARG(tile_w < 65536 && tile_h < 65536, "tile grid too large");
-    hipLaunchKernelGGL(tile_rect_kernel, dim3(gs_cdiv(V, 256)), dim3(256), 0, s, vc, means2d, radii, tile_size, tile_w, tile_h, rect);
-    GS_CHECK_LAUNCH();
-    {
-        const int n_state_words = (int)(bf_state_bytes(V) / 4);
-        hipLaunchKernelGGL(bin_setup_kernel, dim3(gs_cdiv(n_state_words, 256) < 64 ? gs_cdiv(n_state_words, 256) : 64), dim3(256), 0, s, state,
-                           n_state_words, (const long long*)nullptr, 0ll, 0ll, (long long*)nullptr);
-        GS_CHECK_LAUNCH();
-        hipLaunchKernelGGL(emit_chained_kernel, dim3(eblocks), dim3(EM_THREADS), 0, s, vc, (const uint2*)db, (const uint2*)rect, state,
-                           (u64*)((char*)state + 16), eblocks + 1, tile_w, ia, (unsigned)n_isects, (long long*)nullptr);
-        GS_CHECK_LAUNCH();
-    }
+    hipLaunchKernelGGL(emit_chained_kernel, dim3(eblocks), dim3(EM_THREADS), 0, s, vc, (const unsigned*)db, (const uint2*)rb, state,
+                       (u64*)((char*)state + 16), eblocks + 1, tile_w, ia, (unsigned)n_isects,
+                       TileHist{ ttable, tnblocks, (1u << nbits0) - 1u, ic }, (long long*)nullptr);
+    GS_CHECK_LAUNCH();
     uint2* src = ia; uint2* dst = ib;
     for (int pass = 0; pass < npass; ++pass) {
         const int shift = pass * width;
         const int nbits = (tb - shift) < width ? (tb - shift) : width;
+        const XDigit dg{ shift, (1u << nbits) - 1u };
+        auto tile_pass = [&](auto out) {
+            return pass == 0 ? radix_pass_counted<uint2>(ic, U2In{ src }, dg, out, nbits, ttable, s)
+                             : radix_pass<uint2>(ic, U2In{ src }, dg, out, nbits, table, s);
+        };
         if (pass == npass - 1 && tile_ids_sorted != nullptr)
-            rc = radix_pass<uint2>(ic, U2In{ src }, XDigit{ shift, (1u << nbits) - 1u },
-                                   FinalTiles{ tile_ids_sorted, flatten_ids_sorted }, nbits, table, s);
+            rc = tile_pass(FinalTiles{ tile_ids_sorted, flatten_ids_sorted });
         else if (pass == npass - 1)
-            rc = radix_pass<uint2>(ic, U2In{ src }, XDigit{ shift, (1u << nbits) - 1u },
-                                   FinalOut{ (u64*)isect_ids_sorted, flatten_ids_sorted, depths }, nbits, table, s);
+            rc = tile_pass(FinalOut{ (u64*)isect_ids_sorted, flatten_ids_sorted, depths });
         else
-            rc = radix_pass<uint2>(ic, U2In{ src }, XDigit{ shift, (1u << nbits) - 1u }, U2Out{ dst }, nbits, table, s);
+            rc = tile_pass(U2Out{ dst });
         if (rc != GS_OK) return rc;
         uint2* t = src; src = dst; dst = t;
     }
diff --git a/geosplatting_amd/front.py b/geosplatting_amd/front.py
--- a/geosplatting_amd/front.py
+++ b/geosplatting_amd/front.py
@@ -98,6 +98,10 @@
         counts = None
     else:
         V, I, counts = fr.N, int(i_cap), fr.counts
+    rws = None
+    if prepare:
+        rws_bytes = lib.gs_raster_ws_bytes(L.i64(I), V, W, H, tile_size)
+        rws = torch.empty(rws_bytes, dtype=torch.uint8, device=dev)
     if binned is not None:
         flat, offsets = binned
     else:
@@ -105,17 +109,22 @@
         offsets = torch.empty(th * tw, dtype=torch.int32, device=dev)
         bin_bytes = lib.gs_isect_bin_front_ws_bytes(V, L.i64(I), tw, th)
         bin_ws = torch.empty(max(bin_bytes, 1), dtype=torch.uint8, device=dev)
-        L.check(lib.gs_isect_bin_front(V, L.ptr(fr.keys), L.ptr(fr.rects), L.ptr(fr.tile_counts), L.ptr(counts), L.i64(I), fr.key_bits, tw, th,
-                                       L.ptr(flat), L.ptr(offsets), L.ptr(bin_ws), C.c_size_t(bin_bytes),
-                                       L.ptr(status) if counts is not None else None, st), "gs_isect_bin_front")
+        keys = (V, L.ptr(fr.keys), L.ptr(fr.rects), L.ptr(fr.tile_counts), L.ptr(counts), L.i64(I), fr.key_bits, tw, th)
+        st_word = L.ptr(status) if counts is not None else None
+        if prepare:
+            L.check(lib.gs_isect_bin_front_stream(*keys, L.ptr(fr.vis), L.ptr(flat), L.ptr(offsets), L.ptr(bin_ws), C.c_size_t(bin_bytes),
+                                                  L.ptr(rws), C.c_size_t(rws_bytes), st_word, st), "gs_isect_bin_front_stream")
+            L.check(lib.gs_raster_prepare_order(W, H, tile_size, 3, V, L.i64(I), L.ptr(counts), L.ptr(offsets), L.ptr(rws),
+                                                C.c_size_t(rws_bytes), st), "gs_raster_prepare_order")
+        else:
+            L.check(lib.gs_isect_bin_front(*keys, L.ptr(flat), L.ptr(offsets), L.ptr(bin_ws), C.c_size_t(bin_bytes), st_word, st),
+                    "gs_isect_bin_front")
     if not prepare:
         return dict(flatten_ids=flat, isect_offsets=offsets, counts=counts, keys=fr.keys, rects=fr.rects, tile_counts=fr.tile_counts), V, I
-    rws_bytes = lib.gs_raster_ws_bytes(L.i64(I), V, W, H, tile_size)
-    rws = torch.empty(rws_bytes, dtype=torch.uint8, device=dev)
-    if counts is None:
+    if binned is not None and counts is None:
         L.check(lib.gs_raster_prepare_vis(W, H, tile_size, 3, V, L.ptr(fr.vis), L.i64(I), L.ptr(offsets), L.ptr(flat), L.ptr(rws),
                                           C.c_size_t(rws_bytes), st), "gs_raster_prepare_vis")
-    else:
+    elif binned is not None:
         L.check(lib.gs_raster_prepare_vis_cap(W, H, tile_size, 3, V, L.ptr(fr.vis), L.i64(I), L.ptr(counts), L.ptr(offsets), L.ptr(flat),
                                               L.ptr(rws), C.c_size_t(rws_bytes), st), "gs_raster_prepare_vis_cap")
     state = dict(vis_records=fr.vis, flatten_ids=flat, isect_offsets=offsets, raster_ws=rws, counts=counts, keys=fr.keys, rects=fr.rects,
diff --git a/include/geosplat_hip.h b/include/geosplat_hip.h
--- a/include/geosplat_hip.h
+++ b/include/geosplat_hip.h
@@ -300,6 +300,12 @@
 int gs_isect_bin_front(int V_cap, const uint32_t* depth_keys, const uint32_t* tile_rects, const uint32_t* tile_counts,
                        const int64_t* counts_dev, int64_t n_isects_cap, int key_bits, int tile_w, int tile_h, int32_t* flatten_ids_sorted,
                        int32_t* isect_offsets, void* ws, size_t ws_bytes, int64_t* status_dev, void* stream);
+int gs_isect_bin_front_stream(int V_cap, const uint32_t* depth_keys, const uint32_t* tile_rects, const uint32_t* tile_counts,
+                              const int64_t* counts_dev, int64_t n_isects_cap, int key_bits, int tile_w, int tile_h, const float* vis_records,
+                              int32_t* flatten_ids_sorted, int32_t* isect_offsets, void* ws, size_t ws_bytes, void* raster_ws,
+                              size_t raster_ws_bytes, int64_t* status_dev, void* stream);
+int gs_raster_prepare_order(int W, int H, int tile_size, int D, int V, int64_t n_isects, const int64_t* counts_dev,
+                            const int32_t* offsets, void* ws, size_t ws_bytes, void* stream);
 int gs_tail_bwd(int V_cap, const int64_t* counts_dev, const float* means, const float* quats, const float* scales,
                 const float* opacities, const float* normals, const float* kd, const float* ks, const float* viewmat,
                 const float* K, const float* cam_pos, float min_roughness, float max_metallic, int mode, const GsEnv* env,
```

New measurement: 705.5, median of 2. -1.2%, worse.
